# takah29/3d-reconstruction-from-multi-view-exp

Hardware: AMD Instinct MI355X
Metric: BA iterations/sec + residual-Jacobian GObs/s, 1M pts x 100 cams fp64 (higher is better)
Workload: dtype f64

## Files before the change

### 3d-reconstruction-from-multi-view-exp_amd/csrc/mvba.hip

```cpp
#include <dlfcn.h>
#include <hip/hip_runtime.h>
#include <rccl/rccl.h>

#include <algorithm>
#include <atomic>
#include <chrono>
#include <cmath>
#include <cstdlib>
#include <cstring>
#include <thread>
#include <type_traits>
#include <utility>
#include <vector>

#include "mvba_common.h"

namespace mvba {
thread_local std::string g_err;
}
using namespace mvba;

namespace {
struct Rccl {
  void *lib = nullptr;
  int version = 0;
  std::string origin;
  ncclResult_t (*GetVersion)(int *) = nullptr;
  ncclResult_t (*GetUniqueId)(ncclUniqueId *) = nullptr;
  ncclResult_t (*CommInitRank)(ncclComm_t *, int, ncclUniqueId, int) = nullptr;
  ncclResult_t (*CommDestroy)(ncclComm_t) = nullptr;
  ncclResult_t (*AllReduce)(const void *, void *, size_t, ncclDataType_t, ncclRedOp_t, ncclComm_t, hipStream_t) = nullptr;
  ncclResult_t (*AllGather)(const void *, void *, size_t, ncclDataType_t, ncclComm_t, hipStream_t) = nullptr;
  const char *(*GetErrorString)(ncclResult_t) = nullptr;
};
Rccl g_rccl;

int rccl_load() {
  if (g_rccl.lib) return MVBA_OK;
  const char *names[] = {"librccl.so.1", "librccl.so"};
  void *lib = nullptr;
  std::string origin;
  for (const char *n : names)
    if (!lib && (lib = dlopen(n, RTLD_NOW | RTLD_NOLOAD))) origin = std::string(n) + " (already mapped by the process)";
  if (const char *ev = getenv("MVBA_RCCL_LIBRARY"))
    if (!lib && (lib = dlopen(ev, RTLD_NOW | RTLD_GLOBAL))) origin = ev;
  for (const char *n : {"/opt/rocm/lib/librccl.so.1", "librccl.so.1"})
    if (!lib && (lib = dlopen(n, RTLD_NOW | RTLD_GLOBAL))) origin = n;
  if (!lib) return fail(MVBA_ERR_RCCL, std::string("librccl not found: ") + dlerror());
  Rccl r;
  r.lib = lib;
  r.origin = origin;
#define BIND(field, sym)                                                                       \
  if (!(r.field = reinterpret_cast<decltype(r.field)>(dlsym(lib, sym))))                       \
    return fail(MVBA_ERR_RCCL, std::string("librccl (") + origin + ") lacks " + sym)
  BIND(GetVersion, "ncclGetVersion");
  BIND(GetUniqueId, "ncclGetUniqueId");
  BIND(CommInitRank, "ncclCommInitRank");
  BIND(CommDestroy, "ncclCommDestroy");
  BIND(AllReduce, "ncclAllReduce");
  BIND(AllGather, "ncclAllGather");
  BIND(GetErrorString, "ncclGetErrorString");
#undef BIND
  if (r.GetVersion(&r.version) != ncclSuccess) return fail(MVBA_ERR_RCCL, "ncclGetVersion failed");
  const int major = r.version >= 10000 ? r.version / 10000 : r.version / 1000;
  if (major != NCCL_MAJOR)
    return fail(MVBA_ERR_RCCL, "librccl (" + origin + ") is NCCL " + std::to_string(r.version) + ", this library was built against " +
                                   std::to_string(NCCL_VERSION_CODE));
  g_rccl = r;
  return MVBA_OK;
}
}

namespace {

__device__ __forceinline__ double wave_sum(double v) {
#pragma unroll
  for (int off = 32; off > 0; off >>= 1) v += __shfl_down(v, off, 64);
  return v;
}

__device__ __forceinline__ double block_sum(double v, double *s_red ) {
  v = wave_sum(v);
  const int lane = threadIdx.x & 63, w = threadIdx.x >> 6;
  if (lane == 0) s_red[w] = v;
  __syncthreads();
  double t = 0.0;
  if (threadIdx.x == 0) {
    const int nw = (blockDim.x + 63) >> 6;
    for (int i = 0; i < nw; ++i) t += s_red[i];
  }
  return t;
}

__device__ __forceinline__ void load_cams_to_lds(const double *__restrict__ cam15, int m, double f0,
                                                 double *s_cam) {
  for (int k = threadIdx.x; k < m; k += blockDim.x) expand_cam(cam15 + (size_t)k * CAM_IN, f0, s_cam + k * CAM_LDS);
}

__host__ __device__ __forceinline__ size_t strip_offset(int k, int m) {
  return 81 * ((size_t)k * m - (size_t)k * (k - 1) / 2);
}

__device__ __forceinline__ int keep_index(int i, int gauge_axis) {
  if (i < 3) return i;
  return (i + 6 < 12 + gauge_axis) ? i + 6 : i + 7;
}

#define MVBA_CONST_AS __attribute__((address_space(4)))
template <typename T>
__device__ __forceinline__ const T MVBA_CONST_AS *as_const(const T *p) {
#pragma clang diagnostic push
#pragma clang diagnostic ignored "-Wold-style-cast"
  return (const T MVBA_CONST_AS *)p;
#pragma clang diagnostic pop
}

constexpr int REC = 8;
constexpr int LDS_CAMERAS = 646;

#define MVBA_RESID_JAC_ARGS                                                                                                 \
  long long nobs, int m, const double *__restrict__ cam15, const double *__restrict__ X, const int *__restrict__ obs_pt,   \
      const int *__restrict__ cam_idx, const double2 *__restrict__ xy, double f0, const int *__restrict__ tile_start,     \
      int n_tiles, double2 *__restrict__ rec, double *__restrict__ PL, const int *__restrict__ tile_slot,                 \
      double *__restrict__ PLsplit, const double *__restrict__ gcam
struct LossArgs {
  double b;
  double *sqw;
};
template <bool GCAM, int LOSS = LOSS_SQUARED, typename... Robust>
__global__ __launch_bounds__(1024, 4) void k_resid_jac(MVBA_RESID_JAC_ARGS, Robust... robust) {
  extern __shared__ __attribute__((aligned(16))) double smem[];
  double *s_cam = smem;
  const int lane = threadIdx.x & 63, wave = threadIdx.x >> 6, nwave = blockDim.x >> 6;
  double2 *stage = reinterpret_cast<double2 *>(smem + (GCAM ? 0 : ((m * CAM_LDS + 1) & ~1))) + wave * (64 * REC);
  constexpr int CS = 65;
  double *contrib = reinterpret_cast<double *>(stage);
  int *seg_start = reinterpret_cast<int *>(contrib + 9 * CS), *seg_pt = seg_start + 66;
  if (!GCAM) {
    load_cams_to_lds(cam15, m, f0, s_cam);
    __syncthreads();
  }
  for (int tile = blockIdx.x * nwave + wave; tile < n_tiles; tile += gridDim.x * nwave) {
    const int ts0 = tile_start[tile], ts1 = tile_start[tile + 1];
    const bool split = ts0 < 0;
    const int slot = split ? as_const(tile_slot)[tile] : 0;
    const long long wbase = split ? ~ts0 : ts0;
    const int n = (int)((ts1 < 0 ? ~ts1 : ts1) - wbase);
    const long long o = wbase + lane;
    const bool live = lane < n;
    int a = -1;
    double c9[9] = {0, 0, 0, 0, 0, 0, 0, 0, 0};
    if (live) {
      a = obs_pt[o];
      const int k = cam_idx[o];
      const double2 z = xy[o];
      const double *Xa = X + 3 * (size_t)a;
      ObsJ J;
      obs_math(Xa[0], Xa[1], Xa[2], GCAM ? gcam + (size_t)k * CAM_LDS : s_cam + k * CAM_LDS, z.x, z.y, f0, J);
      if constexpr (LOSS != LOSS_SQUARED) {
        const LossArgs la = (robust, ...);
        const double sw = loss_sqrt_w<LOSS>(J.e0 * J.e0 + J.e1 * J.e1, la.b);
        J.e0 *= sw;
        J.e1 *= sw;
#pragma unroll
        for (int rr = 0; rr < 2; ++rr) {
#pragma unroll
          for (int i = 0; i < 3; ++i) J.jx[rr][i] *= sw;
          J.jc[rr][0] *= sw;
#pragma unroll
          for (int i = 6; i < 9; ++i) J.jc[rr][i] *= sw;
        }
        la.sqw[o] = sw;
      }
      double2 *row = stage + lane * REC;
      const int sw = lane & 7;
      row[0 ^ sw] = make_double2(J.jx[0][0], J.jx[1][0]);
      row[1 ^ sw] = make_double2(J.jx[0][1], J.jx[1][1]);
      row[2 ^ sw] = make_double2(J.jx[0][2], J.jx[1][2]);
      row[3 ^ sw] = make_double2(J.jc[0][0], J.jc[1][0]);
      row[4 ^ sw] = make_double2(J.jc[0][6], J.jc[1][6]);
      row[5 ^ sw] = make_double2(J.jc[0][7], J.jc[1][7]);
      row[6 ^ sw] = make_double2(J.jc[0][8], J.jc[1][8]);
      row[7 ^ sw] = make_double2(J.e0, J.e1);
      c9[0] = 2.0 * (J.jx[0][0] * J.jx[0][0] + J.jx[1][0] * J.jx[1][0]);
      c9[1] = 2.0 * (J.jx[0][0] * J.jx[0][1] + J.jx[1][0] * J.jx[1][1]);
      c9[2] = 2.0 * (J.jx[0][0] * J.jx[0][2] + J.jx[1][0] * J.jx[1][2]);
      c9[3] = 2.0 * (J.jx[0][1] * J.jx[0][1] + J.jx[1][1] * J.jx[1][1]);
      c9[4] = 2.0 * (J.jx[0][1] * J.jx[0][2] + J.jx[1][1] * J.jx[1][2]);
      c9[5] = 2.0 * (J.jx[0][2] * J.jx[0][2] + J.jx[1][2] * J.jx[1][2]);
      c9[6] = 2.0 * (J.jx[0][0] * J.e0 + J.jx[1][0] * J.e1);
      c9[7] = 2.0 * (J.jx[0][1] * J.e0 + J.jx[1][1] * J.e1);
      c9[8] = 2.0 * (J.jx[0][2] * J.e0 + J.jx[1][2] * J.e1);
    }
    wave_sync();
#pragma unroll
    for (int q = 0; q < REC; ++q) {
      const int ol = q * 8 + (lane >> 3), pos = lane & 7;
      const double2 v = stage[ol * REC + pos];
      if (ol < n) rec[(wbase + ol) * REC + (pos ^ (ol & 7))] = v;
    }
    wave_sync();
    const int a_prev = __shfl_up(a, 1, 64);
    const bool head = live && (lane == 0 || a != a_prev);
    const unsigned long long heads = __ballot(head);
    const int nseg = __popcll(heads);
#pragma unroll
    for (int q = 0; q < 9; ++q) contrib[q * CS + lane] = c9[q];
    if (head) {
      const int rank = __popcll(heads & ((1ull << lane) - 1ull));
      seg_start[rank] = lane;
      seg_pt[rank] = a;
    }
    if (lane == 0) seg_start[nseg] = n;
    wave_sync();
    const int sl = lane / 9, comp = lane - 9 * sl;
    for (int s0 = 0; s0 < nseg; s0 += 7) {
      const int sg = s0 + sl;
      if (sl < 7 && sg < nseg) {
        const int i0 = seg_start[sg], i1 = seg_start[sg + 1];
        double acc = 0.0;
        for (int i = i0; i < i1; ++i) acc += contrib[comp * CS + i];
        if (split) PLsplit[9 * (size_t)slot + comp] = acc;
        else PL[9 * (size_t)seg_pt[sg] + comp] = acc;
      }
    }
    wave_sync();
  }
}

__global__ void k_sum_split(int n_split, const int4 *__restrict__ splits ,
                            const double *__restrict__ PLsplit, double *__restrict__ PL) {
  const int t = blockIdx.x * blockDim.x + threadIdx.x, sp = t / 9, comp = t - 9 * sp;
  if (sp >= n_split) return;
  const int4 d = splits[sp];
  double v = 0.0;
  for (int q = 0; q < d.z; ++q) v += PLsplit[9 * (size_t)(d.y + q) + comp];
  PL[9 * (size_t)d.x + comp] = v;
}

constexpr int PBS = 16;
constexpr int PACE_STRIDE = 32;
__global__ __launch_bounds__(256) void k_point_inv(long long npts, double c, const double *__restrict__ PL,
                                                   double *__restrict__ PB, int *__restrict__ flag,
                                                   double *__restrict__ Ab, long long nAb, int *__restrict__ prog, long long nprog, int want_r) {
  __shared__ double2 s_out[256 * 8];
  double *s_in = reinterpret_cast<double *>(s_out);
  const long long a0 = (long long)blockIdx.x * 256, a = a0 + threadIdx.x;
  for (long long i = a; i < nAb; i += (long long)gridDim.x * blockDim.x) Ab[i] = 0.0;
  for (long long i = a; i < nprog; i += (long long)gridDim.x * blockDim.x) prog[i] = 0;
  if (a0 >= npts) return;
  const int np = (int)min<long long>(256, npts - a0);
  {
    double t[9];
#pragma unroll
    for (int i = 0; i < 9; ++i) t[i] = PL[9 * a0 + min((int)threadIdx.x + 256 * i, 9 * np - 1)];
#pragma unroll
    for (int i = 0; i < 9; ++i)
      if ((int)threadIdx.x + 256 * i < 9 * np) s_in[threadIdx.x + 256 * i] = t[i];
  }
  __syncthreads();
  double in[9];
#pragma unroll
  for (int i = 0; i < 9; ++i) in[i] = s_in[9 * min((int)threadIdx.x, np - 1) + i];
  __syncthreads();
  if (threadIdx.x < np) {
    const double s = 1.0 + c;
    const double xx = in[0] * s, xy = in[1], xz = in[2], yy = in[3] * s, yz = in[4], zz = in[5] * s;
    const double c00 = yy * zz - yz * yz, c01 = xz * yz - xy * zz, c02 = xy * yz - xz * yy;
    const double det = xx * c00 + xy * c01 + xz * c02;
    if (!(det != 0.0) || !isfinite(det)) atomicOr(flag, 1);
    const double id = 1.0 / det;
    const double i00 = c00 * id, i01 = c01 * id, i02 = c02 * id;
    const double i11 = (xx * zz - xz * xz) * id, i12 = (xy * xz - xx * yz) * id, i22 = (xx * yy - xy * xy) * id;
    const double g0 = in[6], g1 = in[7], g2 = in[8];
    double2 *out = s_out + 8 * threadIdx.x;
    const int sw = threadIdx.x & 7;
    out[0 ^ sw] = make_double2(i00, i01);
    out[1 ^ sw] = make_double2(i02, i11);
    out[2 ^ sw] = make_double2(i12, i22);
    out[3 ^ sw] = make_double2(i00 * g0 + i01 * g1 + i02 * g2, i01 * g0 + i11 * g1 + i12 * g2);
    out[4 ^ sw] = make_double2(i02 * g0 + i12 * g1 + i22 * g2, 1.0);
    if (want_r) {
      const double d0 = i00, q0 = d0 != 0.0 ? 1.0 / d0 : 0.0, l10 = i01 * q0, l20 = i02 * q0;
      const double d1 = i11 - l10 * i01, q1 = d1 != 0.0 ? 1.0 / d1 : 0.0, l21 = (i12 - l20 * i01) * q1;
      const double d2 = i22 - l20 * i02 - l21 * l21 * d1;
      const double a0 = sqrt(fabs(d0)), a1 = sqrt(fabs(d1)), a2 = sqrt(fabs(d2));
      out[4 ^ sw].y = 1.0 + (d0 < 0.0 ? 1.0 : 0.0) + (d1 < 0.0 ? 2.0 : 0.0) + (d2 < 0.0 ? 4.0 : 0.0);
      out[5 ^ sw] = make_double2(a0, l10 * a0);
      out[6 ^ sw] = make_double2(l20 * a0, a1);
      out[7 ^ sw] = make_double2(l21 * a1, a2);
    } else {
      out[5 ^ sw] = out[6 ^ sw] = out[7 ^ sw] = make_double2(0.0, 0.0);
    }
  }
  __syncthreads();
  double2 *dst = reinterpret_cast<double2 *>(PB + PBS * a0);
  for (int e = threadIdx.x; e < 8 * np; e += 256) {
    const int p = e >> 3, sl = e & 7;
    dst[e] = s_out[8 * p + (sl ^ (p & 7))];
  }
}


constexpr int PSTEP = 21;
constexpr int PROW = 7 * 16;
constexpr int PWAVE_LDS = PSTEP * (2 * PROW + 5 * 16);
constexpr int UNIT_STRIDE = 104;
constexpr int SLOT_BUF = PSTEP * (2 * PROW + 3 * 16);
constexpr int SLOT_IDX = 64;
constexpr int SLOT_IDX_RING = 3;
constexpr int PAIRS_LDS = 2 * PWAVE_LDS;
constexpr int SLOT_LDS = 3 * SLOT_BUF + SLOT_IDX_RING * SLOT_IDX * 4;
static_assert(9 * ((SLOT_LDS + 511) / 512 * 512) <= 160 * 1024, "nine waves per CU");

__device__ __forceinline__ void lds_dma16(const void *gsrc, void *lds_wave_uniform) {
  __builtin_amdgcn_global_load_lds(gsrc, (__attribute__((address_space(3))) void *)lds_wave_uniform, 16, 0, 0);
}

struct SlotPace {
  const int *seg_end;
  int *prog;
  int need, nseg, lag;
};
template <bool DIAG, bool BIG, bool SLOTS = false, bool ROBUST = false>
__device__ __forceinline__ void schur_pairs_unit(char *wbuf, const int lane, const long long beg, const int n,
                                                 const int *__restrict__ it_k, const int *__restrict__ it_l,
                                                 const int *__restrict__ it_a, const double2 *__restrict__ rec,
                                                 const double *__restrict__ PB, const double c, const double cu,
                                                 double *__restrict__ out, const int *__restrict__ slot_unit = nullptr,
                                                 const SlotPace pace = SlotPace{nullptr, nullptr, 0, 0, 2},
                                                 const double *__restrict__ sqw = nullptr) {
  static_assert(!(SLOTS && ROBUST), "the slot form has no robust build");
  constexpr int NPS = DIAG ? 5 : 3;
  const int it = lane / 3, cg = lane - 3 * it;
  const int drow = lane / 7, dslot = lane - 7 * drow;
  const int prow = lane / NPS, pslot = lane - NPS * prow;
  const int prow2 = (64 + lane) / 5, pslot2 = (64 + lane) - 5 * prow2;
  const int sel0 = cg == 0 ? 3 : (cg == 1 ? 0 : 4);
  const int sel1 = cg == 0 ? 0 : sel0 + 1, sel2 = cg == 0 ? 0 : sel0 + 2;
  const double al12 = cg == 0 ? 0.0 : 1.0, bx1 = cg == 0 ? 1.0 : 0.0;
  double acc[9][3];
#pragma unroll
  for (int i = 0; i < 9; ++i)
#pragma unroll
    for (int q = 0; q < 3; ++q) acc[i][q] = 0.0;
  double dg[3] = {0.0, 0.0, 0.0}, rb[3] = {0.0, 0.0, 0.0};

  constexpr int LB_OFF = PSTEP * PROW;
  constexpr int PB_OFF = LB_OFF + ((SLOTS && DIAG) ? PSTEP * 16 : PSTEP * PROW);
  constexpr int BUFSZ = SLOTS ? PB_OFF + PSTEP * 16 * NPS : PWAVE_LDS;
  static_assert(!SLOTS || BUFSZ <= SLOT_BUF, "slot form: staging buffer larger than the launch provides");
  constexpr int W_OFF = DIAG ? LB_OFF + PSTEP * 16 : PB_OFF + PSTEP * 16 * NPS;
  static_assert(!ROBUST || (DIAG ? W_OFF + PSTEP * 8 <= PB_OFF : W_OFF + 2 * PSTEP * 8 <= BUFSZ), "robust weights fit the staging buffer");
  int ixk[1][3], ixl[1][3], ixa[1][2];
  int ixw[2] = {0, 0};
  auto load_idx = [&](int s0, int (&xk)[3], int (&xl)[3], int (&xa)[2]) {
    const unsigned last = (unsigned)(min(PSTEP, n - s0) - 1);
    typedef const int __attribute__((address_space(1))) *gint_p;
    auto uni = [](const int *p) {
      const unsigned long long v = (unsigned long long)p;
      const unsigned lo = __builtin_amdgcn_readfirstlane((unsigned)v), hi = __builtin_amdgcn_readfirstlane((unsigned)(v >> 32));
      return (gint_p)(((unsigned long long)hi << 32) | lo);
    };
    typedef const char __attribute__((address_space(1))) *gchar_p;
    auto row_of = [&](int r) {
      unsigned off = min((unsigned)r, last) << 2;
      asm("" : "+v"(off));
      return off;
    };
    auto at = [](gint_p base, unsigned off) { return *(gint_p)((gchar_p)base + off); };
    const gint_p pk = uni(it_k + (beg + s0)), pl = DIAG ? pk : uni(it_l + (beg + s0)), pa = uni(it_a + (beg + s0));
#pragma unroll
    for (int q = 0; q < 3; ++q) {
      const unsigned row = row_of(9 * q + drow);
      xk[q] = at(pk, row);
      if (!DIAG) xl[q] = at(pl, row);
    }
    if (DIAG) xl[0] = at(pk, row_of(lane));
    xa[0] = at(pa, row_of(prow));
    if (DIAG) xa[1] = at(pa, row_of(prow2));
    if (ROBUST) {
      ixw[0] = at(pk, row_of(lane >> 1));
      if (!DIAG) ixw[1] = at(pl, row_of(lane >> 1));
    }
  };
  auto rec_at = [&](int obs, int slot) -> const void * {
    if (BIG) return rec + (size_t)obs * REC + slot;
    return reinterpret_cast<const char *>(rec) + (((unsigned)obs << 7) + ((unsigned)slot << 4));
  };
  auto pb_at = [&](int a, int slot) -> const void * {
    if (BIG) return PB + (size_t)a * PBS + 2 * slot;
    return reinterpret_cast<const char *>(PB) + (((unsigned)a << 7) + ((unsigned)slot << 4));
  };
  auto issue = [&](char *buf, const int (&xk_)[3], const int (&xl_)[3], const int (&xa_)[2]) {
    char *kb = buf, *lb = buf + LB_OFF, *pb_ = buf + PB_OFF;
    const int (&xk)[3] = xk_, (&xl)[3] = xl_, (&xa)[2] = xa_;
    if (lane < 63) {
#pragma unroll
      for (int q = 0; q < 2; ++q) {
        lds_dma16(rec_at(xk[q], dslot), kb + q * (9 * PROW));
        if (!DIAG) lds_dma16(rec_at(xl[q], dslot), lb + q * (9 * PROW));
      }
      if (!DIAG) lds_dma16(pb_at(xa[0], pslot), pb_);
    }
    if (lane < 7 * (PSTEP - 18)) {
      lds_dma16(rec_at(xk[2], dslot), kb + 2 * (9 * PROW));
      if (!DIAG) lds_dma16(rec_at(xl[2], dslot), lb + 2 * (9 * PROW));
    }
    if (DIAG) {
      if (lane < PSTEP) lds_dma16(rec_at(xl[0], 7), lb);
      lds_dma16(pb_at(xa[0], pslot), pb_);
      if (lane < 5 * PSTEP - 64) lds_dma16(pb_at(xa[1], pslot2), pb_ + 1024);
    }
    if (ROBUST && lane < 2 * PSTEP) {
      const char *wsrc = reinterpret_cast<const char *>(sqw) + (lane & 1) * 4;
      __builtin_amdgcn_global_load_lds(wsrc + (size_t)ixw[0] * 8, (__attribute__((address_space(3))) void *)(buf + W_OFF), 4, 0, 0);
      if (!DIAG)
        __builtin_amdgcn_global_load_lds(wsrc + (size_t)ixw[1] * 8, (__attribute__((address_space(3))) void *)(buf + W_OFF + PSTEP * 8), 4, 0, 0);
    }
  };
  auto compute = [&](const char *buf, const int ns) {
    const char *kbuf = buf, *lbuf = buf + LB_OFF, *pbuf = buf + PB_OFF;
    if (it < ns) {
      double swk = 1.0, swl = 1.0;
      if (ROBUST) {
        const double *wl = reinterpret_cast<const double *>(buf + W_OFF);
        swk = wl[it];
        swl = DIAG ? swk : wl[PSTEP + it];
      }
      const double2 *kr = reinterpret_cast<const double2 *>(kbuf + it * PROW);
      const double2 *lr = DIAG ? kr : reinterpret_cast<const double2 *>(lbuf + it * PROW);
      const double *pb = reinterpret_cast<const double *>(pbuf + it * (16 * NPS));
      const double2 kx0 = kr[0], kx1 = kr[1], kx2 = kr[2], kf = kr[3], kw0 = kr[4], kw1 = kr[5], kw2 = kr[6];
      const double2 lx0 = lr[0], lx1 = lr[1], lx2 = lr[2];
      const double i00 = pb[0], i01 = pb[1], i02 = pb[2], i11 = pb[3], i12 = pb[4], i22 = pb[5];
      const double h0x = i00 * lx0.x + i01 * lx1.x + i02 * lx2.x, h0y = i00 * lx0.y + i01 * lx1.y + i02 * lx2.y;
      const double h1x = i01 * lx0.x + i11 * lx1.x + i12 * lx2.x, h1y = i01 * lx0.y + i11 * lx1.y + i12 * lx2.y;
      const double h2x = i02 * lx0.x + i12 * lx1.x + i22 * lx2.x, h2y = i02 * lx0.y + i12 * lx1.y + i22 * lx2.y;
      double t00 = kx0.x * h0x + kx1.x * h1x + kx2.x * h2x, t01 = kx0.x * h0y + kx1.x * h1y + kx2.x * h2y;
      double t10 = kx0.y * h0x + kx1.y * h1x + kx2.y * h2x, t11 = kx0.y * h0y + kx1.y * h1y + kx2.y * h2y;
      double w0 = 0.0, w1 = 0.0;
      const double wgt = (DIAG && SLOTS) ? pb[9] : 1.0;
      if (DIAG) {
        t00 -= SLOTS ? 0.5 * wgt : 0.5;
        t11 -= SLOTS ? 0.5 * wgt : 0.5;
        const double2 e = reinterpret_cast<const double2 *>(lbuf)[it];
        w0 = kx0.x * pb[6] + kx1.x * pb[7] + kx2.x * pb[8] - e.x;
        w1 = kx0.y * pb[6] + kx1.y * pb[7] + kx2.y * pb[8] - e.y;
        if (SLOTS) {
          w0 *= wgt;
          w1 *= wgt;
        }
      }
      const double2 s0v = lr[sel0], s1v = lr[sel1], s2v = lr[sel2];
      const double bxw = ROBUST ? bx1 * swl : bx1;
      const double sx[3] = {s0v.x, al12 * s1v.x + bxw, al12 * s2v.x};
      const double sy[3] = {s0v.y, al12 * s1v.y, al12 * s2v.y + bxw};
#pragma unroll
      for (int q = 0; q < 3; ++q) {
        const double v0 = t00 * sx[q] + t01 * sy[q], v1 = t10 * sx[q] + t11 * sy[q];
        acc[0][q] = fma(kf.y, v1, fma(kf.x, v0, acc[0][q]));
        if (ROBUST) {
          acc[1][q] = fma(swk, v0, acc[1][q]);
          acc[2][q] = fma(swk, v1, acc[2][q]);
        } else {
          acc[1][q] += v0;
          acc[2][q] += v1;
        }
        acc[3][q] = fma(kx0.y, v1, fma(kx0.x, v0, acc[3][q]));
        acc[4][q] = fma(kx1.y, v1, fma(kx1.x, v0, acc[4][q]));
        acc[5][q] = fma(kx2.y, v1, fma(kx2.x, v0, acc[5][q]));
        acc[6][q] = fma(kw0.y, v1, fma(kw0.x, v0, acc[6][q]));
        acc[7][q] = fma(kw1.y, v1, fma(kw1.x, v0, acc[7][q]));
        acc[8][q] = fma(kw2.y, v1, fma(kw2.x, v0, acc[8][q]));
        if (DIAG) {
          if (SLOTS) dg[q] = fma(wgt, sx[q] * sx[q] + sy[q] * sy[q], dg[q]);
          else dg[q] += sx[q] * sx[q] + sy[q] * sy[q];
          rb[q] += sx[q] * w0 + sy[q] * w1;
        }
      }
    }
    asm volatile("s_waitcnt lgkmcnt(0)" ::: "memory");
  };
  bool pacing = SLOTS;
  int seg = 0, seg_stop = pacing ? as_const(pace.seg_end)[0] * PSTEP : 0x7fffffff;
  auto pace_at = [&](const int s0) {
    while (s0 == seg_stop) {
      if (lane == 0) __hip_atomic_fetch_add(pace.prog + PACE_STRIDE * seg, 1, __ATOMIC_RELAXED, __HIP_MEMORY_SCOPE_AGENT);
      ++seg;
      seg_stop = seg < pace.nseg ? as_const(pace.seg_end)[seg] * PSTEP : 0x7fffffff;
      if (seg >= pace.lag && pacing) {
        int tries = 0;
        while (__hip_atomic_fetch_add(pace.prog + PACE_STRIDE * (seg - pace.lag), 0, __ATOMIC_RELAXED, __HIP_MEMORY_SCOPE_AGENT) < pace.need) {
          if (++tries > 1024) { pacing = false; break; }
          __builtin_amdgcn_s_sleep(127);
        }
        if (tries > 0) __builtin_amdgcn_s_setprio(0);
        else __builtin_amdgcn_s_setprio(2);
      }
    }
  };
  if (!SLOTS) {
    load_idx(0, ixk[0], ixl[0], ixa[0]);
    issue(wbuf, ixk[0], ixl[0], ixa[0]);
    if (PSTEP < n) load_idx(PSTEP, ixk[0], ixl[0], ixa[0]);
    for (int s0 = 0, par = 0; s0 < n; s0 += PSTEP, par ^= 1) {
      const int ns = min(PSTEP, n - s0);
      asm volatile("s_waitcnt vmcnt(0)" ::: "memory");
      if (s0 + PSTEP < n) {
        issue(wbuf + (par ^ 1) * BUFSZ, ixk[0], ixl[0], ixa[0]);
        if (s0 + 2 * PSTEP < n) load_idx(s0 + 2 * PSTEP, ixk[0], ixl[0], ixa[0]);
      }
      compute(wbuf + par * BUFSZ, ns);
    }
  } else {
    constexpr int SLOT_OPS = DIAG ? 7 : 8;
    const int nst = n / PSTEP, last_st = nst - 1;
    const unsigned lds0 = (unsigned)(unsigned long long)(__attribute__((address_space(3))) char *)wbuf;
    const unsigned ldsx0 = lds0 + 3 * SLOT_BUF;
    const int *xring = reinterpret_cast<const int *>(wbuf + 3 * SLOT_BUF);
    const int *xbase = it_k + beg * SLOT_IDX;
    static_assert(!SLOTS || !BIG, "the slot form has no 64-bit-offset build");
    auto dma = [&](int row, unsigned slot16, const void *base, unsigned lds) {
      unsigned o;
      asm volatile("s_mov_b32 m0, %4\n\tv_lshl_add_u32 %0, %1, 7, %2\n\tglobal_load_lds_dwordx4 %0, %3" : "=&v"(o) : "v"(row), "v"(slot16), "s"(base), "s"(lds) : "memory");
    };
    const unsigned lane16 = (unsigned)min(lane, 15) << 4;
    auto dma_idx = [&](int st, unsigned ring_off) {
      const int *src = xbase + (size_t)min(st, last_st) * SLOT_IDX;
// ... 1621 lines not shown
  for (int k = threadIdx.x; k < m; k += blockDim.x) {
    const double *Kk = K + 9 * (size_t)k, *Rk = R + 9 * (size_t)k, *tk = t + 3 * (size_t)k;
    double Rt[3][4];
    for (int i = 0; i < 3; ++i) {
      for (int j = 0; j < 3; ++j) Rt[i][j] = Rk[3 * j + i];
      Rt[i][3] = -(Rt[i][0] * tk[0] + Rt[i][1] * tk[1] + Rt[i][2] * tk[2]);
    }
    for (int i = 0; i < 3; ++i)
      for (int j = 0; j < 4; ++j) sP[12 * k + 4 * i + j] = Kk[3 * i] * Rt[0][j] + Kk[3 * i + 1] * Rt[1][j] + Kk[3 * i + 2] * Rt[2][j];
  }
  __syncthreads();
  const long long stride = (long long)gridDim.x * blockDim.x;
  for (long long o = (long long)blockIdx.x * blockDim.x + threadIdx.x; o < nobs; o += stride) {
    const long long a = obs_pt ? obs_pt[o] : o / m;
    const int k = cam_idx ? cam_idx[o] : (int)(o - a * m);
    const double *Xa = X + 3 * a, *P = sP + 12 * k;
    const double p0 = Xa[0] * P[0] + Xa[1] * P[1] + Xa[2] * P[2] + P[3];
    const double p1 = Xa[0] * P[4] + Xa[1] * P[5] + Xa[2] * P[6] + P[7];
    const double p2 = Xa[0] * P[8] + Xa[1] * P[9] + Xa[2] * P[10] + P[11];
    xy[o] = make_double2(p0 / p2, p1 / p2);
  }
}

__global__ __launch_bounds__(256) void k_similarity(long long npts, int m, double *__restrict__ X, double *__restrict__ cam15,
                                                    const double *__restrict__ T13) {
  const double *R0 = T13, *t0 = T13 + 9;
  const double s = T13[12];
  const long long a = (long long)blockIdx.x * blockDim.x + threadIdx.x;
  if (a < npts) {
    double *x = X + 3 * a;
    const double x0 = s * x[0], x1 = s * x[1], x2 = s * x[2];
#pragma unroll
    for (int i = 0; i < 3; ++i) x[i] = x0 * R0[3 * i] + x1 * R0[3 * i + 1] + x2 * R0[3 * i + 2] + t0[i];
  }
  if (a < m) {
    double *c = cam15 + (size_t)a * CAM_IN;
    const double p0 = s * c[3], p1 = s * c[4], p2 = s * c[5];
    double Rn[9];
#pragma unroll
    for (int i = 0; i < 3; ++i) {
#pragma unroll
      for (int j = 0; j < 3; ++j) Rn[3 * i + j] = R0[3 * i] * c[6 + j] + R0[3 * i + 1] * c[9 + j] + R0[3 * i + 2] * c[12 + j];
    }
#pragma unroll
    for (int i = 0; i < 3; ++i) c[3 + i] = p0 * R0[3 * i] + p1 * R0[3 * i + 1] + p2 * R0[3 * i + 2] + t0[i];
#pragma unroll
    for (int i = 0; i < 9; ++i) c[6 + i] = Rn[i];
  }
}

constexpr int IDX_WAVES = 4;

__device__ __forceinline__ int idx_pair_id(int k, int l, int m) { return k * m - k * (k - 1) / 2 + (l - k); }

template <bool GLOBAL>
__global__ __launch_bounds__(64 * IDX_WAVES) void k_idx_count(long long N, int m, int P, const long long *__restrict__ pt_ptr,
                                                              const int *__restrict__ cam_idx, int chunk,
                                                              int *__restrict__ hist, const int *__restrict__ order) {
  extern __shared__ int s_hist_all[];
  const int lane = threadIdx.x & 63, wv = threadIdx.x >> 6;
  const long long w = (long long)blockIdx.x * IDX_WAVES + wv;
  int *s_hist = GLOBAL ? hist + (size_t)w * P : s_hist_all + (size_t)wv * P;
  if (!GLOBAL) {
    for (int q = lane; q < P; q += 64) s_hist[q] = 0;
    wave_sync();
  }
  const long long a0 = w * chunk, a1 = min(N, a0 + chunk);
  for (long long ai = a0; ai < a1; ++ai) {
    const long long a = order ? order[ai] : ai;
    const long long o0 = pt_ptr[a];
    const int d = (int)(pt_ptr[a + 1] - o0);
    for (int i = 0; i < d; ++i) {
      const int k = cam_idx[o0 + i];
      for (int j = i + lane; j < d; j += 64) {
        int *c = s_hist + idx_pair_id(k, cam_idx[o0 + j], m);
        if (GLOBAL) __hip_atomic_store(c, __hip_atomic_load(c, __ATOMIC_RELAXED, __HIP_MEMORY_SCOPE_AGENT) + 1, __ATOMIC_RELAXED, __HIP_MEMORY_SCOPE_AGENT);
        else *c += 1;
      }
      wave_sync();
    }
  }
  if (!GLOBAL)
    for (int q = lane; q < P; q += 64) hist[(size_t)w * P + q] = s_hist[q];
}

__global__ void k_idx_scan(int P, int n_waves, int *__restrict__ hist, long long *__restrict__ cnt) {
  const int q = blockIdx.x * blockDim.x + threadIdx.x;
  if (q >= P) return;
  long long run = 0;
  for (int w = 0; w < n_waves; ++w) {
    const int v = hist[(size_t)w * P + q];
    hist[(size_t)w * P + q] = (int)run;
    run += v;
  }
  cnt[q] = run;
}

template <bool GLOBAL>
__global__ __launch_bounds__(64 * IDX_WAVES) void k_idx_fill(long long N, int m, int P, const long long *__restrict__ pt_ptr,
                                                             const int *__restrict__ cam_idx, int chunk,
                                                             int *__restrict__ hist, const int *__restrict__ S,
                                                             const int *__restrict__ vp_ptr, const long long *__restrict__ vp_off,
                                                             int *__restrict__ it_k, int *__restrict__ it_l, int *__restrict__ it_a,
                                                             const int *__restrict__ order) {
  extern __shared__ int s_hist_all[];
  const int lane = threadIdx.x & 63, wv = threadIdx.x >> 6;
  const long long w = (long long)blockIdx.x * IDX_WAVES + wv;
  int *s_rank = GLOBAL ? hist + (size_t)w * P : s_hist_all + (size_t)wv * P;
  if (!GLOBAL) {
    for (int q = lane; q < P; q += 64) s_rank[q] = hist[(size_t)w * P + q];
    wave_sync();
  }
  const long long a0 = w * chunk, a1 = min(N, a0 + chunk);
  for (long long ai = a0; ai < a1; ++ai) {
    const long long a = order ? order[ai] : ai;
    const long long o0 = pt_ptr[a];
    const int d = (int)(pt_ptr[a + 1] - o0);
    for (int i = 0; i < d; ++i) {
      const int k = cam_idx[o0 + i];
      for (int j = i + lane; j < d; j += 64) {
        const int q = idx_pair_id(k, cam_idx[o0 + j], m);
        int r;
        if (GLOBAL) {
          r = __hip_atomic_load(s_rank + q, __ATOMIC_RELAXED, __HIP_MEMORY_SCOPE_AGENT);
          __hip_atomic_store(s_rank + q, r + 1, __ATOMIC_RELAXED, __HIP_MEMORY_SCOPE_AGENT);
        } else {
          r = s_rank[q];
          s_rank[q] = r + 1;
        }
        const int sq = S[q];
        const long long pos = vp_off[vp_ptr[q] + (r % sq)] + r / sq;
        it_k[pos] = (int)(o0 + i);
        it_l[pos] = (int)(o0 + j);
        it_a[pos] = (int)a;
      }
      wave_sync();
    }
  }
}

__global__ void k_idx_bounds(int VP, int nR, const long long *__restrict__ vp_off, const long long *__restrict__ range_lo,
                             const int *__restrict__ it_a, long long *__restrict__ lo, const int *__restrict__ rank) {
  const long long t = (long long)blockIdx.x * blockDim.x + threadIdx.x;
  if (t >= (long long)VP * (nR + 1)) return;
  const int v = (int)(t / (nR + 1)), r = (int)(t - (long long)v * (nR + 1));
  long long b = vp_off[v], e = vp_off[v + 1];
  const long long key = range_lo[r];
  while (b < e) {
    const long long mid = (b + e) >> 1;
    if ((rank ? rank[it_a[mid]] : it_a[mid]) < key) b = mid + 1;
    else e = mid;
  }
  lo[t] = b;
}

template <bool FILL>
__global__ __launch_bounds__(64) void k_idx_merge(long long n_waves, int nR, int nSeg, long long skew, long long segG,
                                                  const long long *__restrict__ sl_beg, const int *__restrict__ sl_len,
                                                  const long long *__restrict__ range_o0, const int *__restrict__ it_k,
                                                  const int *__restrict__ it_l, const int *__restrict__ it_a,
                                                  const long long *__restrict__ w_beg, int pad_obs, int pad_pt,
                                                  int *__restrict__ w_steps, int *__restrict__ st_k, int *__restrict__ st_l,
                                                  int *__restrict__ st_a, int *__restrict__ seg_end, const long long *__restrict__ pkey) {
  const long long b = blockIdx.x;
  const int lane = threadIdx.x;
  const bool slot = lane < PSTEP;
  long long cur = slot ? sl_beg[b * PSTEP + lane] : 0;
  const long long end = slot ? cur + sl_len[b * PSTEP + lane] : 0;
  const long long o_lo = range_o0[b % nR];
  const long long base = FILL ? w_beg[b] : 0;
  constexpr long long NONE = 1LL << 40;
  int steps = 0, sg = 0;
  auto key_at = [&](long long c) -> long long { return pkey[it_a[c]]; };
  long long k0 = cur < end ? key_at(cur) : NONE, k1 = cur + 1 < end ? key_at(cur + 1) : NONE;
  while (true) {
    long long lo = k0;
#pragma unroll
    for (int off = 32; off > 0; off >>= 1) lo = min(lo, __shfl_xor(lo, off, 64));
    if (FILL && lo < NONE && lane == 0)
      while (sg < nSeg && lo >= o_lo + (sg + 1) * segG) seg_end[b * nSeg + sg++] = steps;
    if (lo >= NONE) break;
    const bool take = k0 < NONE && k0 <= lo + skew;
    if (FILL && slot) {
      const long long o = (base + steps) * PSTEP + lane;
      st_k[o] = take ? (int)(it_k[cur] - o_lo) : pad_obs;
      st_l[o] = take ? (int)(it_l[cur] - o_lo) : pad_obs;
      st_a[o] = take ? it_a[cur] : pad_pt;
    }
    if (take) {
      ++cur;
      k0 = k1;
      k1 = cur + 1 < end ? key_at(cur + 1) : NONE;
    }
    ++steps;
  }
  if (FILL) {
    if (lane == 0)
      while (sg < nSeg) seg_end[b * nSeg + sg++] = steps;
  } else if (lane == 0) {
    w_steps[b] = steps;
  }
}

__global__ void k_idx_interleave(long long n_steps, const int *__restrict__ st_k, const int *__restrict__ st_l, const int *__restrict__ st_a,
                                 int *__restrict__ out) {
  const long long t = (long long)blockIdx.x * blockDim.x + threadIdx.x;
  if (t >= n_steps * SLOT_IDX) return;
  const long long st = t / SLOT_IDX;
  const int e = (int)(t - st * SLOT_IDX), which = e / PSTEP, sl = e - which * PSTEP;
  const int *src = which == 0 ? st_k : (which == 1 ? st_l : st_a);
  out[t] = which < 3 ? src[st * PSTEP + sl] : 0;
}

#include "mvba_cov.h"
#include "mvba_map.h"

}

struct DevBufs {
  std::vector<void *> bufs;
  DevBufs() = default;
  DevBufs(const DevBufs &) = delete;
  DevBufs &operator=(const DevBufs &) = delete;
  ~DevBufs() { release_all(); }
  template <typename T>
  int alloc(T **p, size_t n) {
    const size_t bytes = std::max<size_t>(n, 1) * sizeof(T);
    const hipError_t e = hipMalloc((void **)p, bytes);
    if (e != hipSuccess) {
      size_t fr = 0, tot = 0;
      hipMemGetInfo(&fr, &tot);
      *p = nullptr;
      return fail(MVBA_ERR_HIP, std::string("hipMalloc of ") + std::to_string(bytes) + " bytes: " + hipGetErrorString(e) + " (" + std::to_string(fr >> 20) +
                                    " MiB free of " + std::to_string(tot >> 20) + ")");
    }
    bufs.push_back(*p);
    return MVBA_OK;
  }
  void own(void *q) { bufs.push_back(q); }
  bool forget(void *q) {
    auto it = std::find(bufs.begin(), bufs.end(), q);
    if (it == bufs.end()) return false;
    bufs.erase(it);
    return true;
  }
  template <typename T>
  void release(T *&p) {
    if (p && forget(p)) hipFree(p);
    p = nullptr;
  }
  template <typename T>
  void adopt(DevBufs &from, T *p) {
    if (p && from.forget(p)) bufs.push_back(p);
  }
  void release_all() {
    for (void *q : bufs) hipFree(q);
    bufs.clear();
  }
};

enum { SCHUR_PAIRS = 1, SCHUR_SLOTS = 2, SCHUR_DENSE = 3 };
struct mvba_handle {
  int device = 0;
  hipStream_t stream = nullptr;
  DevBufs mem;
  long long N = 0, nobs = 0;
  int m = 0, gauge_axis = 0, D = 0, ld = 0;
  double f0 = 1.0;
  long long *d_pt_ptr = nullptr;
  int *d_cam = nullptr, *d_obs_pt = nullptr;
  double2 *d_xy = nullptr;
  int *d_tiles = nullptr;
  int *d_tile_slot = nullptr;
  int4 *d_splits = nullptr;
  double *d_PLsplit = nullptr;
  int n_splits = 0;
  int n_tiles = 0;
  bool any_split = false;
  int k1_threads = 512;
  bool use_pairs = true;
  int schur_mode = 2;
  long long n_items = 0, n_items_offdiag = 0, n_slot_items = 0;
  int n_units = 0, rccl_version = 0, q_max = 0, n_waves = 0, slot_nR = 8, slot_nseg = 0;
  long long *d_range_o0 = nullptr;
  int *d_seg_end = nullptr, *d_prog = nullptr;
  bool check_solve = false;
  double check_solve_tol = 1e-8;
  bool gcam = false;
  double *d_cam18 = nullptr, *d_dxi10 = nullptr;
  bool index_on_device = false;
  int4 *d_wdesc = nullptr;
  int *d_it_x = nullptr;
  int *d_wunits = nullptr;
  bool force_big = false;
  int *d_it_k = nullptr, *d_it_l = nullptr, *d_it_a = nullptr, *d_unit_ptr = nullptr, *d_q_ptr = nullptr, *d_q_units = nullptr;
  int4 *d_units = nullptr;
  double *d_partial = nullptr;
  double *d_dense_part = nullptr;
  int *d_dense_obs = nullptr;
  int dense_blocks = 0, dense_tiles = 0;
  double *d_X[2] = {nullptr, nullptr}, *d_cam15[2] = {nullptr, nullptr};
  int cur = 0;
  bool have_params = false, linearized = false, have_trial = false;
  double2 *d_rec = nullptr;
  double *d_PL = nullptr, *d_PB = nullptr;
  double *d_Ab = nullptr, *d_Ared = nullptr, *d_Ztiles = nullptr, *d_Lblk = nullptr, *d_dxi = nullptr, *d_dX = nullptr, *d_lu = nullptr;
  int *d_ipiv = nullptr;
  double *d_partials = nullptr, *d_cost = nullptr, *h_cost = nullptr;
  double *d_mail = nullptr;
  unsigned long long cost_seq = 0;
  bool mail_pending = false;
  int n_partials = 0, cost_grid = 0;
  int *d_flag = nullptr, *h_flag = nullptr;
  unsigned *d_bar = nullptr;
  int n_cu = 1;
  bool chol_onepass = true;
  int trail64_min = 200;
  unsigned barrier_polls = 1u << 22;
  ncclComm_t comm = nullptr;
  mvba_host_allreduce_fn host_ar = nullptr;
  void *host_ar_user = nullptr;
  std::vector<double> host_buf;
  int rank = 0, nranks = 1;
  double *d_allcost = nullptr, *h_allcost = nullptr, *d_sim = nullptr;
  std::vector<double *> snap_slabs;
  long long n_snap = 0;
  int profiling = 0;
  mvba_stats stats{};
  struct Ev { int kid; hipEvent_t a, b; };
  std::vector<Ev> pending;
  std::vector<hipEvent_t> pool;
  double *d_cov_sig = nullptr, *d_cov_panel = nullptr, *d_cov_pts = nullptr, *d_cov_cam = nullptr;
  int loss = LOSS_SQUARED;
  double loss_b = 0.0;
  double *d_sqw = nullptr;
  double2 *d_resid = nullptr;
  double *d_init_cams = nullptr;
  bool mapped = false;
  int n_free = 0, map_ld = 0, map_U = 0;
  std::vector<int> map_col, map_ptr, map_mem;
  int *d_map_col = nullptr, *d_map_ptr = nullptr, *d_map_mem = nullptr;
  double *d_map_x = nullptr, *d_cov_sigv = nullptr;
  int2 *d_map_pairs = nullptr;
  double *d_map_part = nullptr;
  int n_map_pairs = 0, map_nblk = 1;
  int solve_D() const { return mapped ? n_free : D; }
  int solve_ld() const { return mapped ? map_ld : ld; }
};

namespace {

const char *kKernelNames[MVBA_K_COUNT] = {"resid_jac", "point_blocks", "point_inv", "schur",
                                          "allreduce", "solve",        "backsub_cost", "cost"};

struct Timed {
  mvba_handle *h;
  int kid;
  hipEvent_t a = nullptr, b = nullptr;
  bool on = false;
  Timed(mvba_handle *h_, int kid_) : h(h_), kid(kid_) {
    on = kid >= 0 && (h->profiling == 1 || (h->profiling == 2 && (kid == MVBA_K_SCHUR || kid == MVBA_K_RESID_JAC)));
    if (!on) return;
    auto get = [&]() {
      hipEvent_t e;
      if (!h->pool.empty()) { e = h->pool.back(); h->pool.pop_back(); }
      else hipEventCreate(&e);
      return e;
    };
    a = get(); b = get();
    hipEventRecord(a, h->stream);
  }
  ~Timed() {
    if (!on) return;
    hipEventRecord(b, h->stream);
    h->pending.push_back({kid, a, b});
  }
};

void drain_events(mvba_handle *h) {
  for (auto &p : h->pending) {
    float ms = 0.f;
    if (hipEventElapsedTime(&ms, p.a, p.b) == hipSuccess) {
      h->stats.ms[p.kid] += ms;
      h->stats.launches[p.kid] += 1;
    }
    h->pool.push_back(p.a);
    h->pool.push_back(p.b);
  }
  h->pending.clear();
}

int sync_and_drain(mvba_handle *h) {
  MVBA_HIP(hipStreamSynchronize(h->stream));
  drain_events(h);
  return MVBA_OK;
}

inline void cpu_relax() {
#if defined(__x86_64__) && !defined(__HIP_DEVICE_COMPILE__)
  __builtin_ia32_pause();
#endif
}

double *cost_mail(mvba_handle *h) {
  if (h->comm || h->host_ar || h->profiling == 1 || !h->d_mail) return nullptr;
  ++h->cost_seq;
  h->mail_pending = true;
  return h->d_mail;
}

int global_cost(mvba_handle *h, double *E) {
  if (h->mail_pending) {
    h->mail_pending = false;
    volatile unsigned long long *seq = reinterpret_cast<volatile unsigned long long *>(h->h_cost + 2);
    const auto t0 = std::chrono::steady_clock::now();
    bool seen = false;
    for (unsigned spins = 0;; ++spins) {
      if (*seq == h->cost_seq) { seen = true; break; }
      if ((spins & 1023) == 1023 && std::chrono::steady_clock::now() - t0 > std::chrono::seconds(2)) break;
      cpu_relax();
    }
    if (seen) {
      std::atomic_thread_fence(std::memory_order_acquire);
      drain_events(h);
      *E = h->h_cost[0];
      return MVBA_OK;
    }
    int rc = sync_and_drain(h);
    if (rc) return rc;
    *E = h->h_cost[0];
    return MVBA_OK;
  }
  if (h->comm) {
    Timed t(h, MVBA_K_ALLREDUCE);
    ncclResult_t r = g_rccl.AllGather(h->d_cost, h->d_allcost, 2, ncclDouble, h->comm, h->stream);
    if (r != ncclSuccess) return fail(MVBA_ERR_RCCL, std::string("ncclAllGather: ") + g_rccl.GetErrorString(r));
    MVBA_HIP(hipMemcpyAsync(h->h_allcost, h->d_allcost, 2 * sizeof(double) * h->nranks, hipMemcpyDeviceToHost, h->stream));
  } else {
    MVBA_HIP(hipMemcpyAsync(h->h_cost, h->d_cost, 2 * sizeof(double), hipMemcpyDeviceToHost, h->stream));
  }
  int rc = sync_and_drain(h);
  if (rc) return rc;
  if (h->host_ar) {
    std::vector<double> v(2 * (size_t)h->nranks, 0.0);
    v[2 * h->rank] = h->h_cost[0];
    v[2 * h->rank + 1] = (double)*h->h_flag;
    if (h->host_ar(h->host_ar_user, v.data(), (int64_t)v.size())) return fail(MVBA_ERR_RCCL, "host all-reduce callback failed");
    double s = 0.0;
    int fl = 0;
    for (int i = 0; i < h->nranks; ++i) { s += v[2 * i]; fl |= (int)v[2 * i + 1]; }
    *E = s;
    *h->h_flag = fl;
  } else if (h->comm) {
    double s = 0.0;
    int fl = 0;
    for (int i = 0; i < h->nranks; ++i) {
      s += h->h_allcost[2 * i];
      int f;
      memcpy(&f, &h->h_allcost[2 * i + 1], sizeof(int));
      fl |= f;
    }
    *E = s;
    *h->h_flag = fl;
  } else {
    *E = *h->h_cost;
  }
  return MVBA_OK;
}

template <typename... A>
struct LossKernel {
  void (*squared)(A...);
  void (*robust)(A..., LossArgs);
  const void *fn(bool rb) const { return rb ? (const void *)robust : (const void *)squared; }
};
template <typename... A>
LossKernel<A...> loss_kernel(void (*squared)(A...), void (*robust)(A..., LossArgs)) { return {squared, robust}; }

template <typename... A, typename... Args>
void launch_loss(mvba_handle *h, LossKernel<A...> k, dim3 grid, dim3 block, size_t lds, Args... args) {
  if (h->loss != LOSS_SQUARED) hipLaunchKernelGGL(k.robust, grid, block, lds, h->stream, args..., LossArgs{h->loss_b, h->d_sqw});
  else hipLaunchKernelGGL(k.squared, grid, block, lds, h->stream, args...);
}

auto resid_jac_kernel(bool gcam, int loss) {
  if (loss == LOSS_CAUCHY)
    return gcam ? loss_kernel(k_resid_jac<true>, k_resid_jac<true, LOSS_CAUCHY, LossArgs>) : loss_kernel(k_resid_jac<false>, k_resid_jac<false, LOSS_CAUCHY, LossArgs>);
  return gcam ? loss_kernel(k_resid_jac<true>, k_resid_jac<true, LOSS_HUBER, LossArgs>) : loss_kernel(k_resid_jac<false>, k_resid_jac<false, LOSS_HUBER, LossArgs>);
}
auto cost_kernel(bool gcam, int loss) {
  if (loss == LOSS_CAUCHY)
    return gcam ? loss_kernel(k_cost<true>, k_cost<true, LOSS_CAUCHY, LossArgs>) : loss_kernel(k_cost<false>, k_cost<false, LOSS_CAUCHY, LossArgs>);
  return gcam ? loss_kernel(k_cost<true>, k_cost<true, LOSS_HUBER, LossArgs>) : loss_kernel(k_cost<false>, k_cost<false, LOSS_HUBER, LossArgs>);
}
template <int G>
auto backsub_kernel_g(int bt, bool gcam) {
  if (gcam) return loss_kernel(k_backsub<G, 256, true>, k_backsub<G, 256, true, true, LossArgs>);
  if (bt == 1024) return loss_kernel(k_backsub<G, 1024>, k_backsub<G, 1024, false, true, LossArgs>);
  if (bt == 512) return loss_kernel(k_backsub<G, 512>, k_backsub<G, 512, false, true, LossArgs>);
  return loss_kernel(k_backsub<G>, k_backsub<G, 256, false, true, LossArgs>);
}
auto backsub_kernel(int G, int bt, bool gcam) {
  return G == 2 ? backsub_kernel_g<2>(bt, gcam) : (G == 4 ? backsub_kernel_g<4>(bt, gcam) : backsub_kernel_g<8>(bt, gcam));
}
template <int T>
auto dense_kernel_t(bool table) {
  return table ? loss_kernel(k_schur_dense<T, true>, k_schur_dense<T, true, true, LossArgs>)
               : loss_kernel(k_schur_dense<T, false>, k_schur_dense<T, false, true, LossArgs>);
}
auto dense_kernel(int T, bool table) {
  switch (T) {
    case 1: return dense_kernel_t<1>(table);
    case 2: return dense_kernel_t<2>(table);
    case 3: return dense_kernel_t<3>(table);
    case 4: return dense_kernel_t<4>(table);
    case 5: return dense_kernel_t<5>(table);
    case 6: return dense_kernel_t<6>(table);
    case 7: return dense_kernel_t<7>(table);
    case 8: return dense_kernel_t<8>(table);
    case 9: return dense_kernel_t<9>(table);
    case 10: return dense_kernel_t<10>(table);
    case 11: return dense_kernel_t<11>(table);
    default: return dense_kernel_t<12>(table);
  }
}
size_t dense_lds_bytes(int T, int mm) {
  const int CH = dense_ch(T);
  return sizeof(double) * ((size_t)2 * 3 * CH * 16 * T + (size_t)2 * CH * mm * 32) + sizeof(double2) * CH * ((size_t)mm * REC + 8) +
         sizeof(double) * (CH * (size_t)mm + 2 * 3 * CH);
}

size_t k1_lds_bytes(int m, bool gcam, int threads) {
  return (size_t)((gcam ? 0 : ((m * CAM_LDS + 1) & ~1)) + (threads / 64) * 64 * 2 * REC) * sizeof(double);
}
size_t cam_lds_bytes(int m, bool gcam, bool with_dxi) { return gcam ? 0 : (size_t)m * (CAM_LDS + (with_dxi ? DXI_LDS : 0)) * sizeof(double); }

void cam_tables(mvba_handle *h, const double *cam15, const double *dxi) {
  if (h->gcam) hipLaunchKernelGGL(k_cam_tables, dim3((h->m + 255) / 256), dim3(256), 0, h->stream, h->m, cam15, dxi, h->f0, h->d_cam18, h->d_dxi10);
}
int launch_cost(mvba_handle *h, const double *cam15, const double *X) {
  const size_t lds = cam_lds_bytes(h->m, h->gcam, false);
  cam_tables(h, cam15, nullptr);
  launch_loss(h, cost_kernel(h->gcam, h->loss), dim3(h->cost_grid), dim3(lds > 40 * 1024 ? 512 : 256), lds, h->nobs, h->m, cam15, X,
              h->d_obs_pt, h->d_cam, h->d_xy, h->f0, h->d_partials, h->d_cam18);
  double *mail = cost_mail(h);
  const unsigned long long seq = h->cost_seq;
  hipLaunchKernelGGL(k_sum_partials, dim3(1), dim3(1024), 0, h->stream, h->d_partials, h->cost_grid, h->d_cost, h->d_flag, mail, seq);
  MVBA_HIP(hipGetLastError());
  return MVBA_OK;
}

struct CreateKnobs {
  bool schur_set = false;
  bool schur_slots = false, schur_pairs = false, schur_dense = false;
  bool index_host = false, index_global = false;
  bool force_big = false;
  bool chol_launches = false;
  int trail64_min = 200;
  unsigned barrier_polls = 1u << 22;
  bool check_solve = false;
  double check_solve_tol = 1e-8;
  bool timing = false;
};

CreateKnobs read_create_knobs() {
  CreateKnobs k;
  auto is = [](const char *ev, const char *v) { return ev && !strcmp(ev, v); };
  const char *schur = getenv("MVBA_SCHUR");
  k.schur_set = schur != nullptr;
  k.schur_slots = is(schur, "slots");
  k.schur_pairs = is(schur, "pairs");
  k.schur_dense = is(schur, "dense");
  const char *index = getenv("MVBA_INDEX");
  k.index_host = is(index, "host");
  k.index_global = is(index, "global");
  k.force_big = getenv("MVBA_FORCE_BIG") != nullptr;
  k.chol_launches = is(getenv("MVBA_CHOL"), "launches");
  if (const char *ev = getenv("MVBA_TRAIL64_MIN")) k.trail64_min = std::max(0, atoi(ev));
  if (const char *ev = getenv("MVBA_CHOL_BARRIER_POLLS")) k.barrier_polls = (unsigned)std::max(0LL, atoll(ev));
  if (const char *ev = getenv("MVBA_CHECK_SOLVE")) {
    const double v = atof(ev);
    k.check_solve = v != 0.0;
    if (v > 0.0 && v < 1.0) k.check_solve_tol = v;
  }
  k.timing = getenv("MVBA_CREATE_TIMING") != nullptr;
  return k;
}

#include "mvba_create.h"

}

extern "C" {

const char *mvba_version(void) { return "mvba 0.2 (gfx950)"; }
const char *mvba_last_error(void) { return g_err.c_str(); }
const char *mvba_kernel_name(int32_t k) { return (k >= 0 && k < MVBA_K_COUNT) ? kKernelNames[k] : ""; }

int mvba_device_count(int32_t *count) {
  int n = 0;
  hipError_t e = hipGetDeviceCount(&n);
  if (e != hipSuccess) {
    *count = 0;
    return fail(MVBA_ERR_HIP, std::string("hipGetDeviceCount: ") + hipGetErrorString(e));
  }
  *count = n;
  return MVBA_OK;
}

int mvba_create(const mvba_problem *p, mvba_handle **out) { return create_engine(p, LOSS_SQUARED, 0.0, out); }

int mvba_create_robust(const mvba_problem *p, int32_t loss, double scale, mvba_handle **out) {
  if (!p || !out) return fail(MVBA_ERR_BADARG, "null argument");
  if (loss == LOSS_SQUARED) return create_engine(p, LOSS_SQUARED, 0.0, out);
  if (loss != LOSS_HUBER && loss != LOSS_CAUCHY)
    return fail(MVBA_ERR_BADARG, "loss = " + std::to_string(loss) + " is not a loss (0 squared, 1 Huber, 2 Cauchy)");
  if (!(scale > 0.0) || !std::isfinite(scale))
    return fail(MVBA_ERR_BADARG, "loss scale = " + std::to_string(scale) + " must be finite and > 0 for a robust loss");
  if (!(p->f0 > 0.0) || !std::isfinite(p->f0)) return fail(MVBA_ERR_BADARG, "a robust loss needs f0 > 0");
  const double r = scale / p->f0;
  return create_engine(p, loss, r * r, out);
}

void mvba_destroy(mvba_handle *h) {
  if (!h) return;
  hipSetDevice(h->device);
  if (h->stream) hipStreamSynchronize(h->stream);
  if (h->comm) g_rccl.CommDestroy(h->comm);
  h->mem.release_all();
  if (h->h_cost) hipHostFree(h->h_cost);
  if (h->h_allcost) hipHostFree(h->h_allcost);
  for (auto &p : h->pending) { hipEventDestroy(p.a); hipEventDestroy(p.b); }
  for (auto e : h->pool) hipEventDestroy(e);
  if (h->stream) hipStreamDestroy(h->stream);
  delete h;
}

int mvba_set_params(mvba_handle *h, const double *X, const double *f, const double *u, const double *t, const double *R) {
  if (!h || !X || !f || !u || !t || !R) return fail(MVBA_ERR_BADARG, "null argument");
  MVBA_HIP(hipSetDevice(h->device));
  std::vector<double> cam((size_t)h->m * CAM_IN);
  for (int k = 0; k < h->m; ++k) {
    double *c = cam.data() + (size_t)k * CAM_IN;
    c[0] = f[k]; c[1] = u[2 * k]; c[2] = u[2 * k + 1];
    for (int i = 0; i < 3; ++i) c[3 + i] = t[3 * k + i];
    for (int i = 0; i < 9; ++i) c[6 + i] = R[9 * k + i];
  }
  MVBA_HIP(hipMemcpyAsync(h->d_X[h->cur], X, sizeof(double) * 3 * h->N, hipMemcpyHostToDevice, h->stream));
  MVBA_HIP(hipMemcpyAsync(h->d_cam15[h->cur], cam.data(), sizeof(double) * cam.size(), hipMemcpyHostToDevice, h->stream));
  MVBA_HIP(hipStreamSynchronize(h->stream));
  h->have_params = true; h->linearized = false; h->have_trial = false;
  return MVBA_OK;
}

int mvba_get_params(mvba_handle *h, double *X, double *f, double *u, double *t, double *R) {
  if (!h || !X || !f || !u || !t || !R) return fail(MVBA_ERR_BADARG, "null argument");
  if (!h->have_params) return fail(MVBA_ERR_STATE, "no parameters set");
  MVBA_HIP(hipSetDevice(h->device));
  std::vector<double> cam((size_t)h->m * CAM_IN);
  MVBA_HIP(hipMemcpyAsync(X, h->d_X[h->cur], sizeof(double) * 3 * h->N, hipMemcpyDeviceToHost, h->stream));
  MVBA_HIP(hipMemcpyAsync(cam.data(), h->d_cam15[h->cur], sizeof(double) * cam.size(), hipMemcpyDeviceToHost, h->stream));
  MVBA_HIP(hipStreamSynchronize(h->stream));
  for (int k = 0; k < h->m; ++k) {
    const double *c = cam.data() + (size_t)k * CAM_IN;
    f[k] = c[0]; u[2 * k] = c[1]; u[2 * k + 1] = c[2];
    for (int i = 0; i < 3; ++i) t[3 * k + i] = c[3 + i];
    for (int i = 0; i < 9; ++i) R[9 * k + i] = c[6 + i];
  }
  return MVBA_OK;
}

int mvba_apply_similarity(mvba_handle *h, const double *R0, const double *t0, double scale) {
  if (!h || !R0 || !t0) return fail(MVBA_ERR_BADARG, "null argument");
  if (!h->have_params) return fail(MVBA_ERR_STATE, "no parameters set");
  MVBA_HIP(hipSetDevice(h->device));
  double T[13];
  memcpy(T, R0, 9 * sizeof(double));
  memcpy(T + 9, t0, 3 * sizeof(double));
  T[12] = scale;
  if (!h->d_sim) {
    int rc = h->mem.alloc(&h->d_sim, 13);
    if (rc) return rc;
  }
  MVBA_HIP(hipMemcpyAsync(h->d_sim, T, sizeof(T), hipMemcpyHostToDevice, h->stream));
  const long long n = std::max<long long>(h->N, h->m);
  hipLaunchKernelGGL(k_similarity, dim3((unsigned)((n + 255) / 256)), dim3(256), 0, h->stream, h->N, h->m, h->d_X[h->cur],
                     h->d_cam15[h->cur], h->d_sim);
  MVBA_HIP(hipGetLastError());
  MVBA_HIP(hipStreamSynchronize(h->stream));
  h->linearized = false; h->have_trial = false;
  return MVBA_OK;
}

int mvba_cost(mvba_handle *h, double *E) {
  if (!h || !E) return fail(MVBA_ERR_BADARG, "null argument");
  if (!h->have_params) return fail(MVBA_ERR_STATE, "no parameters set");
  MVBA_HIP(hipSetDevice(h->device));
  {
    Timed t(h, MVBA_K_COST);
    int rc = launch_cost(h, h->d_cam15[h->cur], h->d_X[h->cur]);
    if (rc) return rc;
  }
  return global_cost(h, E);
}

namespace {
void launch_resid_jac(mvba_handle *h) {
  const int kt = h->k1_threads;
  cam_tables(h, h->d_cam15[h->cur], nullptr);
  const int wpb = kt / 64;
  const int grid = std::max(1, std::min(2048 * 256 / kt, (h->n_tiles + wpb - 1) / wpb));
  launch_loss(h, resid_jac_kernel(h->gcam, h->loss), dim3(grid), dim3(kt), k1_lds_bytes(h->m, h->gcam, kt), h->nobs, h->m, h->d_cam15[h->cur],
              h->d_X[h->cur], h->d_obs_pt, h->d_cam, h->d_xy, h->f0, h->d_tiles, h->n_tiles, h->d_rec, h->d_PL,
              h->d_tile_slot, h->d_PLsplit, h->d_cam18);
  if (h->n_splits)
    hipLaunchKernelGGL(k_sum_split, dim3((9 * h->n_splits + 255) / 256), dim3(256), 0, h->stream, h->n_splits, h->d_splits,
                       h->d_PLsplit, h->d_PL);
}

void launch_point_inv(mvba_handle *h, double c) {
  const int m = h->m;
  const size_t n9 = 9 * (size_t)m, nA = strip_offset(m, m);
  const long long nAb = (long long)(nA + n9);
  const unsigned grid = (unsigned)std::max<long long>((h->N + 255) / 256, std::min<long long>((nAb + 1023) / 1024, 4096));
  hipLaunchKernelGGL(k_point_inv, dim3(std::max(grid, 1u)), dim3(256), 0, h->stream, h->N, c, h->d_PL, h->d_PB, h->d_flag,
                     h->d_Ab, nAb, h->d_prog, (long long)h->slot_nR * h->slot_nseg * PACE_STRIDE,
                     h->schur_mode == SCHUR_DENSE ? 1 : 0);
}

void launch_schur(mvba_handle *h, double c) {
  const int m = h->m;
  const size_t nA = strip_offset(m, m);
  double *d_A = h->d_Ab, *d_b = h->d_Ab + nA;
  if (h->use_pairs) {
    const bool big = (std::max<long long>(h->nobs, h->N) + 1) * 128LL >= (1LL << 32) || h->force_big;
    if (h->schur_mode == SCHUR_SLOTS) {
      if (h->n_waves)
        hipLaunchKernelGGL(k_schur_slots, dim3(h->n_waves), dim3(64), SLOT_LDS, h->stream, h->d_wdesc,
                           h->d_wunits, h->d_it_x, (const int *)nullptr, (const int *)nullptr, h->d_rec, h->d_PB, c, h->f0, h->d_partial,
                           h->slot_nR, h->d_seg_end, h->d_prog, h->slot_nseg, SLOT_LAG, h->d_range_o0);
    } else if (h->n_units) {
      auto launch = [&](auto kern, auto... robust) {
        hipLaunchKernelGGL(kern, dim3(8 * h->q_max), dim3(64), PAIRS_LDS, h->stream, h->d_units, h->d_q_ptr, h->d_q_units, h->d_it_k, h->d_it_l,
                           h->d_it_a, h->d_rec, h->d_PB, c, h->f0, h->d_partial, robust...);
      };
      if (h->loss != LOSS_SQUARED) launch(big ? k_schur_pairs_big_robust : k_schur_pairs_robust, (const double *)h->d_sqw);
      else launch(big ? k_schur_pairs_big : k_schur_pairs);
    }
    hipLaunchKernelGGL(k_schur_reduce, dim3((unsigned)((long long)m * (m + 1) / 2)), dim3(128), 0, h->stream, m, h->d_unit_ptr,
                       h->d_partial, d_A, d_b);
  } else if (h->schur_mode == SCHUR_DENSE) {
    const int T = (9 * m + 15) / 16;
    launch_loss(h, dense_kernel(T, h->d_dense_obs != nullptr), dim3(h->dense_blocks), dim3(64 * (dense_consumers(T) + dense_ch(T))), dense_lds_bytes(T, m),
                (const double2 *)h->d_rec, (const double *)h->d_PB, (const int *)h->d_dense_obs, (long long)h->N, m, 1.0 / h->f0, h->d_dense_part);
    const long long n_el = (long long)nA + 9 * m;
    hipLaunchKernelGGL(k_schur_dense_finish, dim3((unsigned)((n_el + 3) / 4)), dim3(256), 0, h->stream, m, T, h->dense_blocks,
                       (const double *)h->d_dense_part, c, d_A, d_b);
  }
}

int allreduce_Ab(mvba_handle *h, bool timed) {
  const int m = h->m;
  const size_t n9 = 9 * (size_t)m, nA = strip_offset(m, m);
  if (h->comm) {
    Timed t(h, timed ? MVBA_K_ALLREDUCE : -1);
    ncclResult_t r = g_rccl.AllReduce(h->d_Ab, h->d_Ab, nA + n9, ncclDouble, ncclSum, h->comm, h->stream);
    if (r != ncclSuccess) return fail(MVBA_ERR_RCCL, std::string("ncclAllReduce: ") + g_rccl.GetErrorString(r));
  } else if (h->host_ar) {
    h->host_buf.resize(nA + n9);
    MVBA_HIP(hipMemcpyAsync(h->host_buf.data(), h->d_Ab, sizeof(double) * (nA + n9), hipMemcpyDeviceToHost, h->stream));
    MVBA_HIP(hipStreamSynchronize(h->stream));
    const auto t0 = std::chrono::steady_clock::now();
    if (h->host_ar(h->host_ar_user, h->host_buf.data(), (int64_t)(nA + n9))) return fail(MVBA_ERR_RCCL, "host all-reduce callback failed");
    MVBA_HIP(hipMemcpyAsync(h->d_Ab, h->host_buf.data(), sizeof(double) * (nA + n9), hipMemcpyHostToDevice, h->stream));
    if (timed && h->profiling) {
      h->stats.ms[MVBA_K_ALLREDUCE] += std::chrono::duration<double, std::milli>(std::chrono::steady_clock::now() - t0).count();
      h->stats.launches[MVBA_K_ALLREDUCE] += 1;
    }
  }
  return MVBA_OK;
}

void launch_map_tied(mvba_handle *h, double *M, int ld, int mirror) {
  if (!h->n_map_pairs) return;
  hipLaunchKernelGGL(k_map_tied, dim3(h->n_map_pairs, h->map_nblk), dim3(256), 0, h->stream, h->m, (const double *)h->d_Ab,
                     (const int *)h->d_map_ptr, (const int *)h->d_map_mem, (const int2 *)h->d_map_pairs, h->d_map_part);
  hipLaunchKernelGGL(k_map_tied_finish, dim3((h->n_map_pairs + 255) / 256), dim3(256), 0, h->stream, h->n_map_pairs, h->map_nblk, ld,
                     mirror, (const int2 *)h->d_map_pairs, (const double *)h->d_map_part, M);
}

void launch_factor(mvba_handle *h) {
  const int m = h->m, D = h->solve_D();
  double *d_A = h->d_Ab, *d_b = h->d_Ab + strip_offset(m, m);
  const int ld = h->solve_ld();
  const int ntc = (D + NB - 1) / NB;
  if (h->mapped) {
    const int U = h->map_U, ntu = (U + NB - 1) / NB;
    hipLaunchKernelGGL(k_map_compact, dim3(ntu * (ntu + 1) / 2 + (D + 255) / 256), dim3(256), 0, h->stream, D, ld, m, U, ntu, d_A, d_b,
                       h->d_map_ptr, h->d_map_mem, h->d_Ared, h->d_bar, 1 + 4 * ((D + SBW - 1) / SBW));
    if (U < D)
      hipLaunchKernelGGL(k_map_rows, dim3((D + 63) / 64, D - U), dim3(256), 0, h->stream, D, ld, m, U, d_A, h->d_map_ptr, h->d_map_mem,
                         h->d_Ared);
    launch_map_tied(h, h->d_Ared, ld, 0);
  } else
  hipLaunchKernelGGL(k_compact, dim3(ntc * (ntc + 1) / 2 + (D + 255) / 256), dim3(256), 0, h->stream, D, ld, m, h->gauge_axis, ntc, d_A, d_b,
                     h->d_Ared, h->d_bar, 1 + 4 * ((D + SBW - 1) / SBW));
  for (int jS = 0; jS < D; jS += SBW) {
    const int jE = std::min(jS + SBW, D);
    hipLaunchKernelGGL(k_chol_super, dim3((D + 1 - jE + 63) / 64), dim3(SUPER_THREADS), SUPER_LDS, h->stream, h->d_Ared, ld, D, jS,
                       h->d_Ztiles + (size_t)(jS / NB) * NB * NB, h->d_Lblk + (size_t)(jS / SBW) * SBW * SBW, h->d_flag);
    if (jE < D) {
      const int nt32 = (D + 1 - jE + NB - 1) / NB, nt64 = (D + 1 - jE + TB - 1) / TB;
      if (jE - jS == SBW && nt64 * (nt64 + 1) / 2 >= h->trail64_min)
        hipLaunchKernelGGL(k_chol_trail64, dim3(nt64 * (nt64 + 1) / 2), dim3(256), TRAIL64_LDS, h->stream, h->d_Ared, ld, D, jS, jE);
      else
        hipLaunchKernelGGL(k_chol_trail32, dim3(nt32 * (nt32 + 1) / 2), dim3(256), 0, h->stream, h->d_Ared, ld, D, jS, jE);
    }
  }
}
}

int mvba_linearize(mvba_handle *h) {
  if (!h) return fail(MVBA_ERR_BADARG, "null handle");
  if (!h->have_params) return fail(MVBA_ERR_STATE, "no parameters set");
  MVBA_HIP(hipSetDevice(h->device));
  if (h->nobs) {
    Timed t(h, MVBA_K_RESID_JAC);
    launch_resid_jac(h);
  }
  MVBA_HIP(hipGetLastError());
  h->linearized = true; h->have_trial = false;
  h->stats.n_linearize++;
  return MVBA_OK;
}

namespace {
double *solve_x(mvba_handle *h) { return h->mapped ? h->d_map_x : h->d_dxi; }
void launch_expand(mvba_handle *h) {
  const size_t n9 = 9 * (size_t)h->m;
  if (h->mapped && h->solve_D() > 0)
    hipLaunchKernelGGL(k_map_expand, dim3((unsigned)((n9 + 255) / 256)), dim3(256), 0, h->stream, (int)n9, h->gauge_axis, h->d_map_col,
                       h->d_map_x, h->d_dxi);
}

void launch_solve(mvba_handle *h, bool onepass) {
  const int m = h->m, D = h->solve_D();
  double *d_x = solve_x(h);
  Timed t(h, MVBA_K_SOLVE);
  if (D == 0) {
    hipMemsetAsync(h->d_dxi, 0, sizeof(double) * 9 * (size_t)m, h->stream);
    return;
  }
  launch_factor(h);
  const int ld = h->solve_ld();
  const int S = (D + SBW - 1) / SBW;
  if (onepass && (S == 1 || S < h->n_cu)) {
    const int ngrp = ((S - 1) * SBW + 31) / 32, nbulk = S > 1 ? std::max(1, std::min(h->n_cu - S, ngrp)) : 0;
    hipLaunchKernelGGL(k_chol_backsolve_all<true>, dim3(S + nbulk), dim3(SUPER_THREADS),
                       BACKSOLVE_LDS, h->stream, h->d_Ared, ld, D, m, h->gauge_axis, h->d_Ztiles, h->d_Lblk, d_x, h->d_flag,
                       h->d_bar, h->barrier_polls);
  } else
  for (int jS = ((D - 1) / SBW) * SBW; jS >= 0; jS -= SBW) {
    const int jE = std::min(jS + SBW, D), jE2 = std::min(jE + SBW, D);
    const int nwg = (jE == D) ? 1 : 1 + (jS + 255) / 256;
    hipLaunchKernelGGL(k_chol_backsolve, dim3(nwg), dim3(256), 0, h->stream, h->d_Ared, ld, D, m, h->gauge_axis, h->d_Ztiles,
                       h->d_Lblk + (size_t)(jS / SBW) * SBW * SBW, d_x, jS, jE, jE2);
  }
  launch_expand(h);
}

int launch_lu_solve(mvba_handle *h) {
  const int m = h->m, D = h->solve_D();
  double *d_A = h->d_Ab, *d_b = h->d_Ab + strip_offset(m, m), *d_x = solve_x(h);
  if (!h->d_lu) {
    int rc_ = h->mem.alloc(&h->d_lu, (size_t)h->D * (h->D + 1));
    if (rc_) return rc_;
    rc_ = h->mem.alloc(&h->d_ipiv, (size_t)h->D);
    if (rc_) return rc_;
  }
  MVBA_HIP(hipMemsetAsync(h->d_flag, 0, sizeof(int), h->stream));
  Timed t(h, MVBA_K_SOLVE);
  if (h->mapped) {
    hipLaunchKernelGGL(k_map_full, dim3((D + 1 + 255) / 256, D), dim3(256), 0, h->stream, D, m, d_A, d_b, h->d_map_ptr, h->d_map_mem, h->d_lu);
    launch_map_tied(h, h->d_lu, D + 1, 1);
  } else
  hipLaunchKernelGGL(k_compact_full, dim3((D + 1 + 255) / 256, D), dim3(256), 0, h->stream, D, m, h->gauge_axis, d_A, d_b, h->d_lu);
  for (int j0 = 0; j0 < D; j0 += LU_NB) {
    const int nb = std::min(LU_NB, D - j0), right = D + 1 - (j0 + nb);
    hipLaunchKernelGGL(k_lu_panel, dim3(1), dim3(1024), 0, h->stream, h->d_lu, D, j0, nb, h->d_ipiv, h->d_flag);
    hipLaunchKernelGGL(k_lu_swap, dim3((D + 1 - nb + 255) / 256), dim3(256), 0, h->stream, h->d_lu, D, j0, nb, h->d_ipiv);
    if (right > 0) hipLaunchKernelGGL(k_lu_trsm, dim3((right + 255) / 256), dim3(256), 0, h->stream, h->d_lu, D, j0, nb);
    const int below = D - (j0 + nb);
    if (below > 0)
      hipLaunchKernelGGL(k_lu_gemm, dim3((right + 63) / 64, (below + 63) / 64), dim3(256), 0, h->stream, h->d_lu, D, j0, nb);
  }
  hipLaunchKernelGGL(k_lu_backsub, dim3(1), dim3(1024), 0, h->stream, h->d_lu, D, m, h->gauge_axis, d_x);
  launch_expand(h);
  return MVBA_OK;
}

int launch_tail_and_cost(mvba_handle *h, double *E_trial) {
  const int m = h->m, trial = 1 - h->cur;
  {
    Timed t(h, MVBA_K_BACKSUB_COST);
    hipLaunchKernelGGL(k_update_cams, dim3((m + 63) / 64), dim3(64), 0, h->stream, m, h->d_cam15[h->cur], h->d_dxi,
                       h->d_cam15[trial]);
    if (h->N) {
      const size_t lds = cam_lds_bytes(m, h->gcam, true);
      cam_tables(h, h->d_cam15[h->cur], h->d_dxi);
      const double deg = (double)h->nobs / (double)h->N;
      const int G = deg <= 40.0 ? 2 : (deg <= 100.0 ? 4 : 8);
      const int bt = lds > 80 * 1024 ? 1024 : (lds > 40 * 1024 ? 512 : 256);
      const int nblk = (int)std::min<long long>(4096 * 256 / bt, (h->N * G + bt - 1) / bt);
      launch_loss(h, backsub_kernel(G, bt, h->gcam), dim3(nblk), dim3(bt), lds, h->N, m, h->d_pt_ptr, h->d_cam, h->d_PB, h->d_dxi,
                  h->d_X[h->cur], h->d_cam15[h->cur], h->f0, h->d_X[trial], h->d_dX, h->d_cam18, h->d_dxi10);
    }
    int rc = launch_cost(h, h->d_cam15[trial], h->d_X[trial]);
    if (rc) return rc;
  }
  return global_cost(h, E_trial);
}

int check_solve_residual(mvba_handle *h) {
  const int m = h->m, D = h->solve_D();
  const size_t n9 = 9 * (size_t)m, nA = strip_offset(m, m);
  std::vector<double> Ab(nA + n9), x(n9);
  MVBA_HIP(hipMemcpyAsync(Ab.data(), h->d_Ab, sizeof(double) * (nA + n9), hipMemcpyDeviceToHost, h->stream));
  MVBA_HIP(hipMemcpyAsync(x.data(), h->d_dxi, sizeof(double) * n9, hipMemcpyDeviceToHost, h->stream));
  MVBA_HIP(hipStreamSynchronize(h->stream));
  auto kept = [&](size_t g) { return !((g >= 3 && g <= 8) || g == (size_t)(12 + h->gauge_axis)); };
  std::vector<double> r(n9, 0.0), an(n9, 0.0);
  for (int k = 0; k < m; ++k) {
    const double *Ak = Ab.data() + strip_offset(k, m);
    const int Wk = 9 * (m - k);
    for (int i = 0; i < 9; ++i)
      for (int c = 0; c < Wk; ++c) {
        const size_t gi = 9 * (size_t)k + i, gj = 9 * (size_t)k + c;
        const double a = Ak[(size_t)i * Wk + c];
        r[gi] += a * x[gj]; an[gi] += std::fabs(a * x[gj]);
        if (c >= 9) { r[gj] += a * x[gi]; an[gj] += std::fabs(a * x[gi]); }
      }
  }
  double worst = 0.0;
  if (h->mapped) {
    for (int j = 0; j < D; ++j) {
      double res = 0.0, scale = 0.0;
      for (int q = h->map_ptr[j]; q < h->map_ptr[j + 1]; ++q) {
        const size_t g = (size_t)h->map_mem[q];
        res += Ab[nA + g] - r[g];
        scale += an[g] + std::fabs(Ab[nA + g]);
      }
      worst = std::max(worst, scale > 0.0 ? std::fabs(res) / scale : 0.0);
    }
  } else
  for (size_t g = 0; g < n9; ++g)
    if (kept(g)) {
      const double bg = Ab[nA + g], scale = an[g] + std::fabs(bg);
      worst = std::max(worst, scale > 0.0 ? std::fabs(bg - r[g]) / scale : 0.0);
    }
  if (!(worst <= h->check_solve_tol))
    return fail(MVBA_ERR_STATE, "MVBA_CHECK_SOLVE: the dense solve left a relative residual of " + std::to_string(worst) +
                                    " on the reduced camera system (a stale hand-over in the back-substitution?)");
  return MVBA_OK;
}
}

int mvba_try_step(mvba_handle *h, double c, double *E_trial) {
  if (!h || !E_trial) return fail(MVBA_ERR_BADARG, "null argument");
  if (!h->linearized) return fail(MVBA_ERR_STATE, "try_step before linearize");
  MVBA_HIP(hipSetDevice(h->device));
  {
    Timed t(h, MVBA_K_POINT_INV);
    launch_point_inv(h, c);
  }
  if (h->use_pairs || h->schur_mode == SCHUR_DENSE) {
    Timed t(h, MVBA_K_SCHUR);
    launch_schur(h, c);
  }
  MVBA_HIP(hipGetLastError());
  int rc = allreduce_Ab(h, true);
  if (rc) return rc;
  launch_solve(h, h->chol_onepass);
  MVBA_HIP(hipGetLastError());
  h->stats.n_try_step++;
  rc = launch_tail_and_cost(h, E_trial);
  if (rc) return rc;
  if ((*h->h_flag & 8) && !(*h->h_flag & 1)) {
    MVBA_HIP(hipMemsetAsync(h->d_flag, 0, sizeof(int), h->stream));
    h->chol_onepass = false;
    h->stats.n_barrier_fallback++;
    launch_solve(h, false);
    rc = launch_tail_and_cost(h, E_trial);
    if (rc) return rc;
  }
  if ((*h->h_flag & 2) && !(*h->h_flag & (1 | 8))) {
    rc = launch_lu_solve(h);
    if (rc) return rc;
    h->stats.n_lu_fallback++;
    rc = launch_tail_and_cost(h, E_trial);
    if (rc) return rc;
  }
  if (*h->h_flag) {
    const int fl = *h->h_flag;
    hipMemsetAsync(h->d_flag, 0, sizeof(int), h->stream);
    if (fl & 8) return fail(MVBA_ERR_HIP, "k_chol_backsolve_all: a wait for a progress word timed out twice (is another process holding the CUs?)");
    return fail(MVBA_ERR_SINGULAR, (fl & 1) ? "Singular matrix" : "Singular matrix (reduced camera system)");
  }
  if (h->check_solve) {
    rc = check_solve_residual(h);
    if (rc) return rc;
  }
  h->have_trial = true;
  return MVBA_OK;
}

int mvba_commit(mvba_handle *h) {
  if (!h) return fail(MVBA_ERR_BADARG, "null handle");
  if (!h->have_trial) return fail(MVBA_ERR_STATE, "commit without a trial step");
  h->cur = 1 - h->cur;
  h->have_trial = false; h->linearized = false;
  h->stats.n_commit++;
  return MVBA_OK;
}

int mvba_set_parameter_map(mvba_handle *h, const int32_t *col, int32_t n_free) {
  if (!h) return fail(MVBA_ERR_BADARG, "null handle");
  MVBA_HIP(hipSetDevice(h->device));
  const int m = h->m, n9 = 9 * m;
  auto is_gauge = [&](int g) { return (g >= 3 && g <= 8) || g == 12 + h->gauge_axis; };
  if (!col) {
    h->mapped = false;
    h->have_trial = false;
    return MVBA_OK;
  }
  if (n_free < 0 || n_free > h->D)
    return fail(MVBA_ERR_BADARG, "mvba_set_parameter_map: n_free = " + std::to_string(n_free) + " must be in 0 .. 9 n_images - 7 = " + std::to_string(h->D));
  std::vector<int> cnt(n_free + 1, 0), first(n_free, -1);
  for (int g = 0; g < n9; ++g) {
    const int j = col[g];
    if (j < -1 || j >= n_free)
      return fail(MVBA_ERR_BADARG, "mvba_set_parameter_map: col[" + std::to_string(g) + "] = " + std::to_string(j) + " is neither -1 nor below n_free = " + std::to_string(n_free));
    if (j >= 0 && is_gauge(g))
      return fail(MVBA_ERR_BADARG, "mvba_set_parameter_map: col[" + std::to_string(g) + "] is a gauge slot and must be -1");
    if (j < 0) continue;
    if (first[j] < 0) first[j] = g;
    else if (g % 9 != first[j] % 9 || g % 9 > 2)
      return fail(MVBA_ERR_BADARG, "mvba_set_parameter_map: col[" + std::to_string(g) + "] ties slot " + std::to_string(g) + " to slot " + std::to_string(first[j]) +
                                       " (unknown " + std::to_string(j) + "): only the same intrinsic parameter (f, u or v) of different cameras can be tied");
    ++cnt[j];
  }
  for (int j = 0; j < n_free; ++j)
    if (!cnt[j]) return fail(MVBA_ERR_BADARG, "mvba_set_parameter_map: unknown " + std::to_string(j) + " has no parameter slot");
  bool is_default = n_free == h->D;
  for (int g = 0, j = 0; is_default && g < n9; ++g) is_default = col[g] == (is_gauge(g) ? -1 : j++);
  h->have_trial = false;
  if (is_default) {
    h->mapped = false;
    return MVBA_OK;
  }
  std::vector<int> ptr(n_free + 1, 0), mem;
  for (int j = 0; j < n_free; ++j) ptr[j + 1] = ptr[j] + cnt[j];
  mem.resize(std::max(ptr[n_free], 1));
  {
    std::vector<int> fill(ptr.begin(), ptr.end() - 1);
    for (int g = 0; g < n9; ++g)
      if (col[g] >= 0) mem[fill[col[g]]++] = g;
  }
  int U = 0;
  while (U < n_free && cnt[U] == 1) ++U;
  std::vector<int2> pairs;
  int max_cnt = 1;
  {
    std::vector<int> tied;
    for (int j = 0; j < n_free; ++j)
      if (cnt[j] > 1) { tied.push_back(j); max_cnt = std::max(max_cnt, cnt[j]); }
    for (size_t a = 0; a < tied.size(); ++a)
      for (size_t b = 0; b <= a; ++b) pairs.push_back(make_int2(tied[a], tied[b]));
  }
  const int nblk = std::min(64, (max_cnt + 7) / 8);
  int2 *d_pairs = nullptr;
  double *d_part = nullptr;
  if (!pairs.empty()) {
    int rc = h->mem.alloc(&d_pairs, pairs.size());
    if (!rc) rc = h->mem.alloc(&d_part, pairs.size() * (size_t)nblk);
    if (rc) {
      h->mem.release(d_pairs);
      return rc;
    }
  }
  if (!h->d_map_col) {
    int rc = h->mem.alloc(&h->d_map_col, (size_t)n9);
    if (!rc) rc = h->mem.alloc(&h->d_map_ptr, (size_t)h->D + 1);
    if (!rc) rc = h->mem.alloc(&h->d_map_mem, (size_t)n9);
    if (!rc) rc = h->mem.alloc(&h->d_map_x, (size_t)n9 + 16);
    if (rc) {
      h->mem.release(h->d_map_col); h->mem.release(h->d_map_ptr); h->mem.release(h->d_map_mem); h->mem.release(h->d_map_x);
      h->mem.release(d_pairs); h->mem.release(d_part);
      return rc;
    }
  }
  MVBA_HIP(hipStreamSynchronize(h->stream));
  h->mem.release(h->d_map_pairs);
  h->mem.release(h->d_map_part);
  h->d_map_pairs = d_pairs;
  h->d_map_part = d_part;
  h->n_map_pairs = (int)pairs.size();
  h->map_nblk = nblk;
  if (!pairs.empty()) MVBA_HIP(hipMemcpy(h->d_map_pairs, pairs.data(), sizeof(int2) * pairs.size(), hipMemcpyHostToDevice));
  MVBA_HIP(hipMemcpy(h->d_map_col, col, sizeof(int) * n9, hipMemcpyHostToDevice));
  MVBA_HIP(hipMemcpy(h->d_map_ptr, ptr.data(), sizeof(int) * (n_free + 1), hipMemcpyHostToDevice));
  MVBA_HIP(hipMemcpy(h->d_map_mem, mem.data(), sizeof(int) * mem.size(), hipMemcpyHostToDevice));
  h->map_col.assign(col, col + n9);
  h->map_ptr = ptr;
  h->map_mem = mem;
  h->n_free = n_free;
  h->map_ld = (n_free + 3) & ~3;
  h->map_U = U;
  h->mapped = true;
  return MVBA_OK;
}

int mvba_residuals(mvba_handle *h, double *e) {
  if (!h || !e) return fail(MVBA_ERR_BADARG, "null argument");
  if (!h->have_params) return fail(MVBA_ERR_STATE, "no parameters set");
  MVBA_HIP(hipSetDevice(h->device));
  if (!h->nobs) return MVBA_OK;
  if (!h->d_resid) {
    int rc = h->mem.alloc(&h->d_resid, h->nobs);
    if (rc) return rc;
  }
  const size_t lds = h->gcam ? 0 : (size_t)h->m * CAM_LDS * sizeof(double);
  cam_tables(h, h->d_cam15[h->cur], nullptr);
  const unsigned grid = (unsigned)std::min<long long>(4096, (h->nobs + 255) / 256);
  hipLaunchKernelGGL(h->gcam ? k_residuals<true> : k_residuals<false>, dim3(grid), dim3(256), lds, h->stream, h->nobs, h->m,
                     (const double *)h->d_cam15[h->cur], (const double *)h->d_X[h->cur], (const int *)h->d_obs_pt, (const int *)h->d_cam,
                     (const double2 *)h->d_xy, h->f0, h->d_resid, (const double *)h->d_cam18);
  MVBA_HIP(hipGetLastError());
  MVBA_HIP(hipMemcpyAsync(e, h->d_resid, sizeof(double2) * h->nobs, hipMemcpyDeviceToHost, h->stream));
  MVBA_HIP(hipStreamSynchronize(h->stream));
  return MVBA_OK;
}

int mvba_covariance(mvba_handle *h, double *point_cov, double *cam_cov, double *cam_cov_full, double *timings_ms) {
  if (!h) return fail(MVBA_ERR_BADARG, "null handle");
  if (h->loss != LOSS_SQUARED)
    return fail(MVBA_ERR_BADARG, "mvba_covariance: the covariance is defined for the squared loss only (this engine has a robust loss)");
  if (!h->have_params) return fail(MVBA_ERR_STATE, "no parameters set");
  MVBA_HIP(hipSetDevice(h->device));
  const int m = h->m, D = h->solve_D(), ld = h->solve_ld(), nt = (D + NB - 1) / NB;
  const size_t n_sig = sig_block(m, m, m);
  auto free_cov = [&]() {
    for (double **q : {&h->d_cov_sig, &h->d_cov_panel, &h->d_cov_pts, &h->d_cov_cam}) h->mem.release(*q);
  };
  int local_rc = MVBA_OK;
  if (!h->d_cov_sig || !h->d_cov_panel || !h->d_cov_pts || !h->d_cov_cam) {
    free_cov();
    local_rc = h->mem.alloc(&h->d_cov_sig, n_sig);
    if (!local_rc) local_rc = h->mem.alloc(&h->d_cov_panel, 2 * (size_t)h->D * NB);
    if (!local_rc) local_rc = h->mem.alloc(&h->d_cov_pts, 6 * (size_t)h->N);
    if (!local_rc) local_rc = h->mem.alloc(&h->d_cov_cam, 81 * (size_t)m);
    if (local_rc) free_cov();
  }
  hipEvent_t ev[5] = {};
  struct EvFree { hipEvent_t *e; ~EvFree() { for (int i = 0; i < 5; ++i) if (e[i]) hipEventDestroy(e[i]); } } ev_free{ev};
  for (auto &e : ev)
    if (!local_rc && hipEventCreate(&e) != hipSuccess) local_rc = fail(MVBA_ERR_HIP, "hipEventCreate failed");
  const int mv = (D + 6) / 9 + 1;
  if (!local_rc && h->mapped && D > 0 && !h->d_cov_sigv) local_rc = h->mem.alloc(&h->d_cov_sigv, n_sig);
  const bool sharded = h->comm || h->host_ar;
  if (local_rc && !sharded) return local_rc;
  const std::string local_err = local_rc ? g_err : std::string();
  double *d_b = h->d_Ab + strip_offset(m, m);
  if (!local_rc) {
    MVBA_HIP(hipEventRecord(ev[0], h->stream));
    if (h->nobs) launch_resid_jac(h);
    h->linearized = true; h->have_trial = false;
    launch_point_inv(h, 0.0);
    launch_schur(h, 0.0);
    MVBA_HIP(hipGetLastError());
  } else {
    MVBA_HIP(hipMemsetAsync(d_b + 3, 0xFF, sizeof(double), h->stream));
  }
  {
    int rc = allreduce_Ab(h, false);
    if (rc) return rc;
  }
  if (sharded) {
    double mark = 0.0;
    MVBA_HIP(hipMemcpyAsync(&mark, d_b + 3, sizeof(double), hipMemcpyDeviceToHost, h->stream));
    MVBA_HIP(hipStreamSynchronize(h->stream));
    if (local_rc) return fail(local_rc, local_err);
    if (std::isnan(mark))
      return fail(MVBA_ERR_HIP, "mvba_covariance: another rank could not allocate its covariance buffers (or the reduced system is not finite)");
  }
  MVBA_HIP(hipEventRecord(ev[1], h->stream));
  if (D > 0) launch_factor(h);
  MVBA_HIP(hipEventRecord(ev[2], h->stream));
  if (D > 0)
  hipLaunchKernelGGL(k_cov_assemble, dim3(nt), dim3(256), 0, h->stream, h->d_Ared, ld, D, (const double *)h->d_Ztiles,
                     (const double *)h->d_Lblk);
  double *panel[2] = {h->d_cov_panel, h->d_cov_panel + (size_t)D * NB};
  for (int J = nt - 1; J >= 0; --J) {
    const int grid = (nt - 1 - J) + (J >= 1 ? nt - J : 0);
    if (grid)
      hipLaunchKernelGGL(k_cov_trtri, dim3(grid), dim3(256), 0, h->stream, h->d_Ared, ld, D, nt, J, (const double *)panel[J & 1],
                         panel[(J + 1) & 1]);
  }
  MVBA_HIP(hipMemsetAsync(h->d_cov_sig, 0, sizeof(double) * n_sig, h->stream));
  if (h->mapped) {
    if (D > 0) {
      hipLaunchKernelGGL(k_cov_lauum, dim3(nt * (nt + 1) / 2), dim3(256), 0, h->stream, (const double *)h->d_Ared, ld, D, nt, mv,
                         h->gauge_axis, h->d_cov_sigv);
      hipLaunchKernelGGL(k_map_cov_expand, dim3((unsigned)((81 * m + 255) / 256), m), dim3(256), 0, h->stream, m, mv, h->gauge_axis,
                         (const int *)h->d_map_col, (const double *)h->d_cov_sigv, h->d_cov_sig);
    }
  } else
  hipLaunchKernelGGL(k_cov_lauum, dim3(nt * (nt + 1) / 2), dim3(256), 0, h->stream, (const double *)h->d_Ared, ld, D, nt, m,
                     h->gauge_axis, h->d_cov_sig);
  MVBA_HIP(hipEventRecord(ev[3], h->stream));
  if (h->N && point_cov) {
    const double pairs = h->N ? 0.5 * ((double)h->nobs / (double)h->N) * ((double)h->nobs / (double)h->N + 1.0) : 0.0;
    const int G = pairs > 48.0 ? 64 : (pairs > 24.0 ? 32 : (pairs > 12.0 ? 16 : 8));
    const unsigned grid = (unsigned)std::min<long long>(8192, (h->N * G + 255) / 256);
    auto kern = G == 64 ? k_point_cov<64> : (G == 32 ? k_point_cov<32> : (G == 16 ? k_point_cov<16> : k_point_cov<8>));
    hipLaunchKernelGGL(kern, dim3(grid), dim3(256), 0, h->stream, h->N, m, (const long long *)h->d_pt_ptr, (const int *)h->d_cam,
                       (const double2 *)h->d_rec, (const double *)h->d_PL, (const double *)h->d_cov_sig, 1.0 / h->f0, h->d_cov_pts,
                       h->d_flag);
  }
  if (cam_cov)
    hipLaunchKernelGGL(k_cov_cam_diag, dim3((unsigned)((81LL * m + 255) / 256)), dim3(256), 0, h->stream, m,
                       (const double *)h->d_cov_sig, h->d_cov_cam);
  MVBA_HIP(hipGetLastError());
  MVBA_HIP(hipEventRecord(ev[4], h->stream));
  int fl = 0;
  MVBA_HIP(hipMemcpyAsync(&fl, h->d_flag, sizeof(int), hipMemcpyDeviceToHost, h->stream));
  MVBA_HIP(hipStreamSynchronize(h->stream));
  if (fl) {
    MVBA_HIP(hipMemsetAsync(h->d_flag, 0, sizeof(int), h->stream));
    MVBA_HIP(hipStreamSynchronize(h->stream));
    if (fl & (1 | COV_FLAG_POINT)) return fail(MVBA_ERR_SINGULAR, "Singular matrix (a point block E_a is singular: a point seen once, or without parallax)");
    return fail(MVBA_ERR_SINGULAR, "Singular matrix (the undamped reduced camera system is not positive definite)");
  }
  if (timings_ms)
    for (int i = 0; i < 4; ++i) {
      float ms = 0.f;
      MVBA_HIP(hipEventElapsedTime(&ms, ev[i], ev[i + 1]));
      timings_ms[i] = ms;
    }
  if (point_cov && h->N) MVBA_HIP(hipMemcpy(point_cov, h->d_cov_pts, sizeof(double) * 6 * h->N, hipMemcpyDeviceToHost));
  if (cam_cov) MVBA_HIP(hipMemcpy(cam_cov, h->d_cov_cam, sizeof(double) * 81 * m, hipMemcpyDeviceToHost));
  if (cam_cov_full) {
    std::vector<double> strip((size_t)SIG_BS * m);
    const size_t n9 = 9 * (size_t)m;
    for (int k = 0; k < m; ++k) {
      MVBA_HIP(hipMemcpy(strip.data(), h->d_cov_sig + sig_block(k, k, m), sizeof(double) * SIG_BS * (m - k), hipMemcpyDeviceToHost));
      for (int l = k; l < m; ++l) {
        const double *b = strip.data() + (size_t)SIG_BS * (l - k);
        for (int i = 0; i < 9; ++i)
          for (int j = 0; j < 9; ++j) {
            const double v = 2.0 * b[9 * i + j];
            cam_cov_full[(9 * (size_t)k + i) * n9 + 9 * (size_t)l + j] = v;
            cam_cov_full[(9 * (size_t)l + j) * n9 + 9 * (size_t)k + i] = v;
          }
      }
    }
  }
  return MVBA_OK;
}

namespace {
constexpr int SNAP_SLAB = 8;
size_t snap_stride(const mvba_handle *h) { return (3 * (size_t)h->N + (size_t)CAM_IN * h->m + 1) & ~(size_t)1; }
}

int mvba_snapshot(mvba_handle *h) {
  if (!h) return fail(MVBA_ERR_BADARG, "null handle");
  if (!h->have_params) return fail(MVBA_ERR_STATE, "no parameters set");
  MVBA_HIP(hipSetDevice(h->device));
  const size_t stride = snap_stride(h);
  const size_t slab = (size_t)(h->n_snap / SNAP_SLAB);
  if (slab >= h->snap_slabs.size()) {
    double *p = nullptr;
    int rc = h->mem.alloc(&p, stride * SNAP_SLAB);
    if (rc) return rc;
    h->snap_slabs.push_back(p);
  }
  double *dst = h->snap_slabs[slab] + stride * (size_t)(h->n_snap % SNAP_SLAB);
  MVBA_HIP(hipMemcpyAsync(dst, h->d_X[h->cur], sizeof(double) * 3 * h->N, hipMemcpyDeviceToDevice, h->stream));
  MVBA_HIP(hipMemcpyAsync(dst + 3 * h->N, h->d_cam15[h->cur], sizeof(double) * CAM_IN * h->m, hipMemcpyDeviceToDevice, h->stream));
  h->n_snap++;
  return MVBA_OK;
}

int mvba_snapshot_count(mvba_handle *h, int64_t *n) {
  if (!h || !n) return fail(MVBA_ERR_BADARG, "null argument");
  *n = h->n_snap;
  return MVBA_OK;
}

int mvba_snapshot_read(mvba_handle *h, int64_t i, double *X, double *f, double *u, double *t, double *R) {
  if (!h || !X || !f || !u || !t || !R) return fail(MVBA_ERR_BADARG, "null argument");
  if (i < 0 || i >= h->n_snap) return fail(MVBA_ERR_BADARG, "no such log entry");
  MVBA_HIP(hipSetDevice(h->device));
  const double *src = h->snap_slabs[(size_t)(i / SNAP_SLAB)] + snap_stride(h) * (size_t)(i % SNAP_SLAB);
  std::vector<double> cam((size_t)h->m * CAM_IN);
  MVBA_HIP(hipMemcpyAsync(X, src, sizeof(double) * 3 * h->N, hipMemcpyDeviceToHost, h->stream));
  MVBA_HIP(hipMemcpyAsync(cam.data(), src + 3 * h->N, sizeof(double) * cam.size(), hipMemcpyDeviceToHost, h->stream));
  MVBA_HIP(hipStreamSynchronize(h->stream));
  for (int k = 0; k < h->m; ++k) {
    const double *c = cam.data() + (size_t)k * CAM_IN;
    f[k] = c[0]; u[2 * k] = c[1]; u[2 * k + 1] = c[2];
    for (int q = 0; q < 3; ++q) t[3 * k + q] = c[3 + q];
    for (int q = 0; q < 9; ++q) R[9 * k + q] = c[6 + q];
  }
  return MVBA_OK;
}

int mvba_snapshot_restore(mvba_handle *h, int64_t i) {
  if (!h) return fail(MVBA_ERR_BADARG, "null handle");
  if (i < 0 || i >= h->n_snap) return fail(MVBA_ERR_BADARG, "no such log entry");
  MVBA_HIP(hipSetDevice(h->device));
  const double *src = h->snap_slabs[(size_t)(i / SNAP_SLAB)] + snap_stride(h) * (size_t)(i % SNAP_SLAB);
  MVBA_HIP(hipMemcpyAsync(h->d_X[h->cur], src, sizeof(double) * 3 * h->N, hipMemcpyDeviceToDevice, h->stream));
  MVBA_HIP(hipMemcpyAsync(h->d_cam15[h->cur], src + 3 * h->N, sizeof(double) * CAM_IN * h->m, hipMemcpyDeviceToDevice, h->stream));
  h->have_params = true; h->linearized = false; h->have_trial = false;
  return MVBA_OK;
}

int mvba_snapshot_clear(mvba_handle *h) {
  if (!h) return fail(MVBA_ERR_BADARG, "null handle");
  h->n_snap = 0;
  return MVBA_OK;
}

int mvba_set_profiling(mvba_handle *h, int32_t enabled) {
  if (!h) return fail(MVBA_ERR_BADARG, "null handle");
  h->profiling = enabled == 2 ? 2 : (enabled != 0);
  return MVBA_OK;
}

int mvba_get_stats(mvba_handle *h, mvba_stats *out) {
  if (!h || !out) return fail(MVBA_ERR_BADARG, "null argument");
  MVBA_HIP(hipSetDevice(h->device));
  int rc = sync_and_drain(h);
  if (rc) return rc;
  *out = h->stats;
  return MVBA_OK;
}

int mvba_get_info(mvba_handle *h, int64_t *out8) {
  if (!h || !out8) return fail(MVBA_ERR_BADARG, "null argument");
  out8[0] = h->n_items;
  out8[1] = h->n_items_offdiag;
  out8[2] = h->n_units;
  out8[3] = h->schur_mode;
  out8[4] = h->rccl_version;
  out8[5] = NCCL_VERSION_CODE;
  out8[6] = h->nranks;
  out8[7] = h->schur_mode == SCHUR_SLOTS ? h->n_slot_items : 0;
  return MVBA_OK;
}

int mvba_reset_stats(mvba_handle *h) {
  if (!h) return fail(MVBA_ERR_BADARG, "null handle");
  MVBA_HIP(hipSetDevice(h->device));
  int rc = sync_and_drain(h);
  if (rc) return rc;
  h->stats = mvba_stats{};
  return MVBA_OK;
}

int mvba_comm_unique_id(void *id128) {
  if (!id128) return fail(MVBA_ERR_BADARG, "null argument");
  static_assert(sizeof(ncclUniqueId) == 128, "ncclUniqueId size");
  if (int rc = rccl_load()) return rc;
  ncclUniqueId id;
  ncclResult_t r = g_rccl.GetUniqueId(&id);
  if (r != ncclSuccess) return fail(MVBA_ERR_RCCL, std::string("ncclGetUniqueId: ") + g_rccl.GetErrorString(r));
  memcpy(id128, &id, 128);
  return MVBA_OK;
}

int mvba_comm_init(mvba_handle *h, const void *id128, int32_t rank, int32_t n_ranks) {
  if (!h || !id128 || n_ranks < 1 || rank < 0 || rank >= n_ranks) return fail(MVBA_ERR_BADARG, "bad comm arguments");
  MVBA_HIP(hipSetDevice(h->device));
  if (int rc = rccl_load()) return rc;
  ncclUniqueId id;
  memcpy(&id, id128, 128);
  ncclResult_t r = g_rccl.CommInitRank(&h->comm, n_ranks, id, rank);
  if (r != ncclSuccess) return fail(MVBA_ERR_RCCL, std::string("ncclCommInitRank: ") + g_rccl.GetErrorString(r));
  h->rank = rank; h->nranks = n_ranks;
  h->rccl_version = g_rccl.version;
  int rc = h->mem.alloc(&h->d_allcost, 2 * (size_t)n_ranks);
  if (rc) return rc;
  MVBA_HIP(hipHostMalloc((void **)&h->h_allcost, 2 * sizeof(double) * n_ranks));
  return MVBA_OK;
}

int mvba_comm_init_host(mvba_handle *h, int32_t rank, int32_t n_ranks, mvba_host_allreduce_fn fn, void *user) {
  if (!h || !fn || n_ranks < 1 || rank < 0 || rank >= n_ranks) return fail(MVBA_ERR_BADARG, "bad comm arguments");
  if (h->comm) return fail(MVBA_ERR_STATE, "handle already has an RCCL communicator");
  h->host_ar = fn; h->host_ar_user = user;
  h->rank = rank; h->nranks = n_ranks;
  return MVBA_OK;
}

int mvba_debug_read(mvba_handle *h, int32_t which, double *out, int64_t capacity, int64_t *n) {
  if (!h || !n) return fail(MVBA_ERR_BADARG, "null argument");
  MVBA_HIP(hipSetDevice(h->device));
  const size_t n9 = 9 * (size_t)h->m;
  long long cnt = 0;
  switch (which) {
    case MVBA_BUF_RESIDUAL: cnt = 2 * h->nobs; break;
    case MVBA_BUF_JX: cnt = 6 * h->nobs; break;
    case MVBA_BUF_JC: cnt = 18 * h->nobs; break;
    case MVBA_BUF_E: cnt = 6 * h->N; break;
    case MVBA_BUF_DP: cnt = 3 * h->N; break;
    case MVBA_BUF_A_FULL: cnt = n9 * n9; break;
    case MVBA_BUF_B_FULL: cnt = n9; break;
    case MVBA_BUF_DXI: cnt = n9; break;
    case MVBA_BUF_DX: case MVBA_BUF_TRIAL_X: cnt = 3 * h->N; break;
    case MVBA_BUF_TRIAL_CAM: cnt = (long long)CAM_IN * h->m; break;
    case MVBA_BUF_INDEX_K: case MVBA_BUF_INDEX_L: case MVBA_BUF_INDEX_A:
      cnt = h->schur_mode == SCHUR_SLOTS ? h->n_slot_items : (h->schur_mode == SCHUR_PAIRS ? h->n_items : 0);
      break;
    case MVBA_BUF_INDEX_SEG: cnt = h->schur_mode == SCHUR_SLOTS ? (long long)h->n_waves * h->slot_nseg : 0; break;
    case MVBA_BUF_WEIGHT: cnt = h->nobs; break;
    default: return fail(MVBA_ERR_BADARG, "unknown buffer id");
  }
  *n = cnt;
  if (!out) return MVBA_OK;
  if (capacity < cnt) return fail(MVBA_ERR_BADARG, "output buffer too small");
  MVBA_HIP(hipStreamSynchronize(h->stream));
  auto d2h = [&](const void *src, size_t bytes) { return hipMemcpy(out, src, bytes, hipMemcpyDeviceToHost); };
  if (which == MVBA_BUF_RESIDUAL || which == MVBA_BUF_JX || which == MVBA_BUF_JC) {
    std::vector<double> r((size_t)2 * REC * h->nobs);
    MVBA_HIP(hipMemcpy(r.data(), h->d_rec, sizeof(double) * r.size(), hipMemcpyDeviceToHost));
    std::vector<double> sw;
    if (h->loss != LOSS_SQUARED && which == MVBA_BUF_JC) {
      sw.resize(h->nobs);
      MVBA_HIP(hipMemcpy(sw.data(), h->d_sqw, sizeof(double) * sw.size(), hipMemcpyDeviceToHost));
    }
    for (long long o = 0; o < h->nobs; ++o) {
      const double cu = sw.empty() ? 1.0 / h->f0 : sw[o] / h->f0;
      const double *q = r.data() + (size_t)o * 2 * REC;
      if (which == MVBA_BUF_RESIDUAL) {
        out[2 * o] = q[14]; out[2 * o + 1] = q[15];
      } else if (which == MVBA_BUF_JX) {
        for (int rr = 0; rr < 2; ++rr) for (int i = 0; i < 3; ++i) out[6 * o + 3 * rr + i] = q[2 * i + rr];
      } else {
        double *jc = out + 18 * o;
        for (int rr = 0; rr < 2; ++rr) {
          jc[9 * rr + 0] = q[6 + rr];
          jc[9 * rr + 1] = rr == 0 ? cu : 0.0;
          jc[9 * rr + 2] = rr == 1 ? cu : 0.0;
          for (int i = 0; i < 3; ++i) jc[9 * rr + 3 + i] = -q[2 * i + rr];
          for (int i = 0; i < 3; ++i) jc[9 * rr + 6 + i] = q[8 + 2 * i + rr];
        }
      }
    }
  } else if (which == MVBA_BUF_WEIGHT) {
    if (h->loss != LOSS_SQUARED) MVBA_HIP(d2h(h->d_sqw, sizeof(double) * h->nobs));
    else for (long long o = 0; o < h->nobs; ++o) out[o] = 1.0;
  } else if (which == MVBA_BUF_E || which == MVBA_BUF_DP) {
    std::vector<double> pl(9 * (size_t)h->N);
    MVBA_HIP(hipMemcpy(pl.data(), h->d_PL, sizeof(double) * pl.size(), hipMemcpyDeviceToHost));
    for (long long a = 0; a < h->N; ++a) {
      if (which == MVBA_BUF_E) for (int i = 0; i < 6; ++i) out[6 * a + i] = pl[9 * a + i];
      else for (int i = 0; i < 3; ++i) out[3 * a + i] = pl[9 * a + 6 + i];
    }
  } else if (which == MVBA_BUF_A_FULL) {
    const int m = h->m;
    std::vector<double> pk(strip_offset(m, m));
    MVBA_HIP(hipMemcpy(pk.data(), h->d_Ab, sizeof(double) * pk.size(), hipMemcpyDeviceToHost));
    for (size_t r = 0; r < n9; ++r)
      for (size_t cc = 0; cc < n9; ++cc) {
        const size_t lo = std::min(r, cc), hi = std::max(r, cc);
        const int k = (int)(lo / 9), l = (int)(hi / 9);
        const size_t rr = (k == l) ? r : lo, c2 = (k == l) ? cc : hi;
        out[r * n9 + cc] = pk[strip_offset(k, m) + (rr - 9 * k) * (size_t)(9 * (m - k)) + (c2 - 9 * k)];
      }
  } else if (which == MVBA_BUF_B_FULL) {
    MVBA_HIP(d2h(h->d_Ab + strip_offset(h->m, h->m), sizeof(double) * cnt));
  } else if (which == MVBA_BUF_DXI) {
    MVBA_HIP(d2h(h->d_dxi, sizeof(double) * cnt));
  } else if (which == MVBA_BUF_DX) {
    MVBA_HIP(d2h(h->d_dX, sizeof(double) * cnt));
  } else if (which == MVBA_BUF_TRIAL_X) {
    MVBA_HIP(d2h(h->d_X[1 - h->cur], sizeof(double) * cnt));
  } else if (which == MVBA_BUF_TRIAL_CAM) {
    MVBA_HIP(d2h(h->d_cam15[1 - h->cur], sizeof(double) * cnt));
  } else if (which >= MVBA_BUF_INDEX_K && which <= MVBA_BUF_INDEX_SEG) {
    if (h->schur_mode == SCHUR_SLOTS && which != MVBA_BUF_INDEX_SEG) {
      const long long n_steps = cnt / PSTEP;
      std::vector<int> tmp((size_t)n_steps * SLOT_IDX);
      if (cnt) MVBA_HIP(hipMemcpy(tmp.data(), h->d_it_x, sizeof(int) * tmp.size(), hipMemcpyDeviceToHost));
      const int off = which == MVBA_BUF_INDEX_K ? 0 : (which == MVBA_BUF_INDEX_L ? PSTEP : 2 * PSTEP);
      for (long long st = 0; st < n_steps; ++st)
        for (int sl = 0; sl < PSTEP; ++sl) out[st * PSTEP + sl] = (double)tmp[(size_t)st * SLOT_IDX + off + sl];
      return MVBA_OK;
    }
    const int *src = which == MVBA_BUF_INDEX_K ? h->d_it_k : (which == MVBA_BUF_INDEX_L ? h->d_it_l : (which == MVBA_BUF_INDEX_A ? h->d_it_a : h->d_seg_end));
    std::vector<int> tmp((size_t)cnt);
    if (cnt) MVBA_HIP(hipMemcpy(tmp.data(), src, sizeof(int) * tmp.size(), hipMemcpyDeviceToHost));
    for (long long i = 0; i < cnt; ++i) out[i] = (double)tmp[i];
  }
  return MVBA_OK;
}

int mvba_project(const double *X, int64_t n_points, const double *K, const double *R, const double *t, int32_t n_images,
                 const int64_t *pt_ptr, const int32_t *cam_idx, int64_t n_obs, double *xy, int32_t device) {
  if (!X || !K || !R || !t || !xy) return fail(MVBA_ERR_BADARG, "null argument");
  if (n_points < 0 || n_images < 1 || n_obs < 0 || (pt_ptr && !cam_idx)) return fail(MVBA_ERR_BADARG, "bad sizes");
  if (!pt_ptr && n_obs != n_points * (int64_t)n_images) return fail(MVBA_ERR_BADARG, "dense grid needs n_obs = n_points * n_images");
  if (n_points >= (1LL << 31)) return fail(MVBA_ERR_BADARG, "n_points must be < 2^31");
  if ((size_t)n_images * 12 * sizeof(double) > 160 * 1024 - 256) return fail(MVBA_ERR_BADARG, "too many cameras for the LDS camera table (max 1704)");
  if (n_obs == 0) return MVBA_OK;
  if (device >= 0) MVBA_HIP(hipSetDevice(device));
  std::vector<int> obs_pt;
  if (pt_ptr) {
    if (pt_ptr[0] != 0 || pt_ptr[n_points] != n_obs) return fail(MVBA_ERR_BADARG, "pt_ptr does not span n_obs");
    obs_pt.resize(n_obs);
    for (int64_t a = 0; a < n_points; ++a)
      for (int64_t o = pt_ptr[a]; o < pt_ptr[a + 1]; ++o) {
        if (cam_idx[o] < 0 || cam_idx[o] >= n_images) return fail(MVBA_ERR_BADARG, "cam_idx out of range");
        obs_pt[o] = (int)a;
      }
  }
  double *dX = nullptr, *dK = nullptr, *dR = nullptr, *dt = nullptr;
  double2 *dxy = nullptr;
  int *dpt = nullptr, *dcam = nullptr;
  DevBufs tmp;
#define PRJ(x) do { hipError_t e_ = (x); if (e_ != hipSuccess) return fail(MVBA_ERR_HIP, std::string(#x) + ": " + hipGetErrorString(e_)); } while (0)
  PRJ(hipMalloc((void **)&dX, sizeof(double) * 3 * std::max<int64_t>(n_points, 1))); tmp.own(dX);
  PRJ(hipMalloc((void **)&dK, sizeof(double) * 9 * n_images)); tmp.own(dK);
  PRJ(hipMalloc((void **)&dR, sizeof(double) * 9 * n_images)); tmp.own(dR);
  PRJ(hipMalloc((void **)&dt, sizeof(double) * 3 * n_images)); tmp.own(dt);
  PRJ(hipMalloc((void **)&dxy, sizeof(double2) * n_obs)); tmp.own(dxy);
  PRJ(hipMemcpy(dX, X, sizeof(double) * 3 * n_points, hipMemcpyHostToDevice));
  PRJ(hipMemcpy(dK, K, sizeof(double) * 9 * n_images, hipMemcpyHostToDevice));
  PRJ(hipMemcpy(dR, R, sizeof(double) * 9 * n_images, hipMemcpyHostToDevice));
  PRJ(hipMemcpy(dt, t, sizeof(double) * 3 * n_images, hipMemcpyHostToDevice));
  if (pt_ptr) {
    PRJ(hipMalloc((void **)&dpt, sizeof(int) * n_obs)); tmp.own(dpt);
    PRJ(hipMalloc((void **)&dcam, sizeof(int) * n_obs)); tmp.own(dcam);
    PRJ(hipMemcpy(dpt, obs_pt.data(), sizeof(int) * n_obs, hipMemcpyHostToDevice));
    PRJ(hipMemcpy(dcam, cam_idx, sizeof(int) * n_obs, hipMemcpyHostToDevice));
  }
  const int lds = (int)(sizeof(double) * 12 * n_images);
  PRJ(hipFuncSetAttribute((const void *)k_project_obs, hipFuncAttributeMaxDynamicSharedMemorySize, lds));
  const int grid = (int)std::max<int64_t>(1, std::min<int64_t>(2048, (n_obs + 255) / 256));
  hipLaunchKernelGGL(k_project_obs, dim3(grid), dim3(256), lds, 0, (long long)n_obs, n_images, dX, dK, dR, dt, dpt, dcam, dxy);
  PRJ(hipGetLastError());
  PRJ(hipMemcpy(xy, dxy, sizeof(double2) * n_obs, hipMemcpyDeviceToHost));
#undef PRJ
  return MVBA_OK;
}

int mvba_host_obs_math(const double *X3, const double *cam15, const double *xy2, double f0, double *out26) {
  if (!X3 || !cam15 || !xy2 || !out26) return fail(MVBA_ERR_BADARG, "null argument");
  alignas(16) double c[CAM_LDS];
  expand_cam(cam15, f0, c);
  ObsJ J;
  obs_math(X3[0], X3[1], X3[2], c, xy2[0], xy2[1], f0, J);
  out26[0] = J.e0; out26[1] = J.e1;
  for (int r = 0; r < 2; ++r) for (int i = 0; i < 3; ++i) out26[2 + 3 * r + i] = J.jx[r][i];
  for (int r = 0; r < 2; ++r) for (int i = 0; i < 9; ++i) out26[8 + 9 * r + i] = J.jc[r][i];
  return MVBA_OK;
}

}

#include "mvba_init.h"
#include "mvba_twoview.h"
```

### 3d-reconstruction-from-multi-view-exp_amd/csrc/mvba_create.h

```cpp

__global__ __launch_bounds__(256) void k_xy_from_planes(const double2 *__restrict__ planes, long long N, int m, double2 *__restrict__ xy) {
  const long long a = (long long)blockIdx.x * 256 + threadIdx.x;
  const int k = blockIdx.y;
  if (a < N) xy[a * m + k] = planes[(long long)k * N + a];
}

#define CR(x) do { int rc_ = (x); if (rc_) return rc_; } while (0)
#define CRH(x) do { hipError_t e_ = (x); if (e_ != hipSuccess) return fail(MVBA_ERR_HIP, std::string(#x) + ": " + hipGetErrorString(e_)); } while (0)

struct CreateTimer {
  bool on;
  std::chrono::steady_clock::time_point t_last = std::chrono::steady_clock::now();
  void lap(const char *what) {
    if (!on) return;
    const auto now = std::chrono::steady_clock::now();
    fprintf(stderr, "mvba_create: %-28s %8.1f ms\n", what, std::chrono::duration<double, std::milli>(now - t_last).count());
    t_last = now;
  }
};

int validate_problem(const mvba_problem *p, std::vector<int> &obs_pt) {
  if (p->n_points < 0 || p->n_images < 2 || p->n_obs < 0 || !p->pt_ptr || (p->n_obs && (!p->cam_idx || !p->xy)))
    return fail(MVBA_ERR_BADARG, "bad problem sizes or null arrays (need n_images >= 2)");
  if (p->gauge_axis != 0 && p->gauge_axis != 1) return fail(MVBA_ERR_BADARG, "gauge_axis must be 0 or 1");
// ... 302 lines not shown
  }
  for (const std::vector<int> *src : {&diag_lists, &off_lists})
    for (size_t first = 0; first < src->size(); first += PSTEP) {
      for (int sl = 0; sl < PSTEP; ++sl) wl.push_back(first + sl < src->size() ? (*src)[first + sl] : -1);
      sw.w_isdiag.push_back(src == &diag_lists);
    }
  const long long n_waves = sw.n_waves = (long long)sw.w_isdiag.size() * nR;
  ix.wdesc.assign(n_waves, make_int4(0, 0, 0, 0));
  ix.wunits.assign((size_t)n_waves * PSTEP, -1);
  sw.w_steps.assign(n_waves, 0);
  sw.w_beg.assign(n_waves + 1, 0);
  sw.sl_beg.assign((size_t)n_waves * PSTEP, 0);
  sw.sl_len.assign((size_t)n_waves * PSTEP, 0);
  for (long long b = 0; b < n_waves; ++b) {
    const int *vs = wl.data() + (size_t)(b / nR) * PSTEP;
    const int r = (int)(b % nR);
    for (int sl = 0; sl < PSTEP; ++sl) {
      const int id = vs[sl] >= 0 ? uid[(size_t)vs[sl] * nR + r] : -1;
      ix.wunits[(size_t)b * PSTEP + sl] = id;
      if (id < 0) continue;
      sw.sl_beg[(size_t)b * PSTEP + sl] = ((long long)ix.units[id].y << 32) | (unsigned)ix.units[id].x;
      sw.sl_len[(size_t)b * PSTEP + sl] = ix.units[id].z;
    }
  }
  for (int r = 0; r < nR; ++r)
    sw.nSeg = std::max<long long>(sw.nSeg, (in.p->pt_ptr[plan.R.lo[r + 1]] - in.p->pt_ptr[plan.R.lo[r]] + SLOT_SEG - 1) / SLOT_SEG);
  ix.seg_end.assign((size_t)n_waves * sw.nSeg, 0);
  ix.slot_nseg = sw.nSeg;
  return sw;
}

int upload_range_o0(const IndexInput &in, const PointRanges &R, DevBufs &engine, SchurIndex &ix) {
  std::vector<long long> ro0(R.nR);
  for (int r = 0; r < R.nR; ++r) ro0[r] = in.p->pt_ptr[R.lo[r]];
  CR(engine.alloc(&ix.d_range_o0, (size_t)R.nR));
  CRH(hipMemcpy(ix.d_range_o0, ro0.data(), sizeof(long long) * R.nR, hipMemcpyHostToDevice));
  return MVBA_OK;
}

int place_slot_steps(const SchurPlan &plan, SlotWaves &sw, const SchurIndex &ix, long long &total_steps) {
  for (long long b = 0; b < sw.n_waves; ++b) sw.w_beg[b + 1] = sw.w_beg[b] + sw.w_steps[b];
  total_steps = sw.w_beg[sw.n_waves];
  if (total_steps * PSTEP >= (1LL << 40)) return fail(MVBA_ERR_BADARG, "too many (point, camera pair) items");
  const size_t need = (size_t)total_steps * PSTEP * 12 + (size_t)total_steps * SLOT_IDX * 4 + ix.seg_end.size() * 4;
  size_t fr = 0, tot = 0;
  if (hipMemGetInfo(&fr, &tot) == hipSuccess && need > fr)
    return fail(MVBA_ERR_BADARG, "the slot-form Schur index needs " + std::to_string(need >> 20) + " MiB (" + std::to_string(total_steps * PSTEP) + " step rows for " +
                                     std::to_string(plan.L.T) + " items: " + std::to_string(plan.R.nR) + " ranges, skew " + std::to_string(SLOT_SKEW) + "), " +
                                     std::to_string(fr >> 20) + " MiB of device memory are free: use MVBA_SCHUR=pairs");
  return MVBA_OK;
}

void finish_slot_waves(const PointRanges &R, const SlotWaves &sw, long long total_steps, SchurIndex &ix) {
  const int nR = R.nR;
  std::vector<int> live(nR, 0);
  for (long long b = 0; b < sw.n_waves; ++b) live[b % nR] += sw.w_steps[b] > 0;
  for (long long b = 0; b < sw.n_waves; ++b) {
    const long long beg = sw.w_beg[b];
    ix.wdesc[b] = make_int4((int)(beg & 0xffffffffLL), (int)(beg >> 32), (int)sw.w_steps[b],
                            (sw.w_isdiag[b / nR] ? 1 : 0) | (live[b % nR] << 8));
  }
  ix.n_waves = (int)sw.n_waves;
  ix.slot_nR = nR;
  ix.n_slot_items = total_steps * PSTEP;
}

int count_pairs_host(const IndexInput &in, std::vector<long long> &cnt) {
  const mvba_problem *p = in.p;
  const int m = in.m, n_thr = in.n_thr;
  on_threads(n_thr, [&](int tid) {
    for (long long a = 0; a < in.N; ++a) {
      const int *cb = p->cam_idx + p->pt_ptr[a];
      const int d = (int)(p->pt_ptr[a + 1] - p->pt_ptr[a]);
      for (int i = 0; i < d; ++i) {
        if (cb[i] % n_thr != tid) continue;
        long long *row = cnt.data() + pair_id(m, cb[i], cb[i]) - cb[i];
        for (int j = i; j < d; ++j) row[cb[j]]++;
      }
    }
  });
  return MVBA_OK;
}

int build_index_host(const IndexInput &in, const SchurPlan &plan, DevBufs &engine, SchurIndex &ix, CreateTimer &timer) {
  const mvba_problem *p = in.p;
  const PairLists &L = plan.L;
  const PointRanges &R = plan.R;
  const long long N = in.N, P = in.P;
  const int m = in.m, n_thr = in.n_thr, nR = R.nR;
  std::vector<int> &it_k = ix.it_k, &it_l = ix.it_l, &it_a = ix.it_a;
  it_k.resize(L.T); it_l.resize(L.T); it_a.resize(L.T);
  {
    std::vector<long long> run(P, 0);
    on_threads(n_thr, [&](int tid) {
      for (long long a = 0; a < N; ++a) {
        const long long o0 = p->pt_ptr[a];
        const int *cb = p->cam_idx + o0;
        const int d = (int)(p->pt_ptr[a + 1] - o0);
        for (int i = 0; i < d; ++i) {
          if (cb[i] % n_thr != tid) continue;
          const long long rowp = pair_id(m, cb[i], cb[i]) - cb[i];
          for (int j = i; j < d; ++j) {
            const long long q = rowp + cb[j], r = run[q]++;
            const int sI = (int)(r % L.S[q]);
            const long long pos = L.vp_off[L.vp_ptr[q] + sI] + r / L.S[q];
            it_k[pos] = (int)(o0 + i); it_l[pos] = (int)(o0 + j); it_a[pos] = (int)a;
          }
        }
      }
    });
  }
  timer.lap("items sorted by pair");
  std::vector<int> uid;
  number_units(in, plan, [&](int v, int r) {
    auto before = [](int a, long long key) { return (long long)a < key; };
    return (long long)(std::lower_bound(it_a.data() + L.vp_off[v], it_a.data() + L.vp_off[v + 1], R.lo[r], before) - it_a.data());
  }, ix, uid);
  timer.lap("units");
  if (plan.mode == SCHUR_SLOTS) {
    SlotWaves sw = make_slot_waves(in, plan, uid, ix);
    const int nSeg = sw.nSeg;
    std::vector<int> st_k, st_l, st_a;
    auto merge = [&](long long b, long long base, bool fill) {
      const int r = (int)(b % nR);
      long long cur[PSTEP], end[PSTEP];
      for (int sl = 0; sl < PSTEP; ++sl) {
        cur[sl] = sw.sl_beg[(size_t)b * PSTEP + sl];
        end[sl] = cur[sl] + sw.sl_len[(size_t)b * PSTEP + sl];
      }
      long long steps = 0;
      const long long o_lo = p->pt_ptr[R.lo[r]];
      int sg = 0;
      auto key_of = [&](int sl) { return p->pt_ptr[it_a[cur[sl]]]; };
      while (true) {
        long long lo = -1;
        for (int sl = 0; sl < PSTEP; ++sl)
          if (cur[sl] < end[sl] && (lo < 0 || key_of(sl) < lo)) lo = key_of(sl);
        if (fill && lo >= 0)
          while (sg < nSeg && lo >= o_lo + (sg + 1) * SLOT_SEG) ix.seg_end[(size_t)b * nSeg + sg++] = (int)steps;
        if (lo < 0) break;
        for (int sl = 0; sl < PSTEP; ++sl) {
          const bool take = cur[sl] < end[sl] && key_of(sl) <= lo + SLOT_SKEW;
          if (fill) {
            const long long o = (base + steps) * PSTEP + sl;
            if (take) { st_k[o] = (int)(it_k[cur[sl]] - o_lo); st_l[o] = (int)(it_l[cur[sl]] - o_lo); st_a[o] = it_a[cur[sl]]; }
            else { st_k[o] = st_l[o] = 0; st_a[o] = (int)N; }
          }
          if (take) ++cur[sl];
        }
        ++steps;
      }
      if (fill)
        while (sg < nSeg) ix.seg_end[(size_t)b * nSeg + sg++] = (int)steps;
      return steps;
    };
    CR(upload_range_o0(in, R, engine, ix));
    on_threads(n_thr, [&](int tid) {
      for (long long b = tid; b < sw.n_waves; b += n_thr) sw.w_steps[b] = merge(b, 0, false);
    });
    timer.lap("slot merge (count)");
    long long total_steps = 0;
    CR(place_slot_steps(plan, sw, ix, total_steps));
    st_k.resize(total_steps * PSTEP); st_l.resize(total_steps * PSTEP); st_a.resize(total_steps * PSTEP);
    on_threads(n_thr, [&](int tid) {
      for (long long b = tid; b < sw.n_waves; b += n_thr)
        if (sw.w_steps[b]) merge(b, sw.w_beg[b], true);
    });
    timer.lap("slot merge (fill)");
    finish_slot_waves(R, sw, total_steps, ix);
    it_k.swap(st_k); it_l.swap(st_l); it_a.swap(st_a);
  } else {
    build_work_queues(in, plan, uid, ix);
  }
  return MVBA_OK;
}

struct DeviceIndexBuild {
  DevBufs mem;
  bool hist_lds = true;
  int idx_chunk = 32;
  long long idx_waves = 0;
  size_t idx_lds = 0;
  int *d_hist = nullptr;
  long long *d_cnt = nullptr;
};

int count_pairs_device(const IndexInput &in, const CreateKnobs &knobs, DeviceIndexBuild &dv, std::vector<long long> &cnt) {
  const long long N = in.N, P = in.P;
  dv.hist_lds = (size_t)P * sizeof(int) * IDX_WAVES <= 150 * 1024 && !knobs.index_global;
  const long long max_idx_waves = dv.hist_lds ? 4096 : std::max<long long>(IDX_WAVES, std::min<long long>(4096, (2LL << 30) / (4 * P)));
  dv.idx_chunk = (int)std::max<long long>(32, (N + max_idx_waves - 1) / max_idx_waves);
  dv.idx_waves = ((N + dv.idx_chunk - 1) / dv.idx_chunk + IDX_WAVES - 1) / IDX_WAVES * IDX_WAVES;
  dv.idx_lds = dv.hist_lds ? P * sizeof(int) * IDX_WAVES : 0;
  CR(dv.mem.alloc(&dv.d_hist, (size_t)dv.idx_waves * P));
  CR(dv.mem.alloc(&dv.d_cnt, (size_t)P));
  if (dv.hist_lds) {
    CRH(hipFuncSetAttribute((const void *)k_idx_count<false>, hipFuncAttributeMaxDynamicSharedMemorySize, (int)dv.idx_lds));
    CRH(hipFuncSetAttribute((const void *)k_idx_fill<false>, hipFuncAttributeMaxDynamicSharedMemorySize, (int)dv.idx_lds));
  } else {
    CRH(hipMemsetAsync(dv.d_hist, 0, sizeof(int) * (size_t)dv.idx_waves * P, in.stream));
  }
  hipLaunchKernelGGL(dv.hist_lds ? k_idx_count<false> : k_idx_count<true>, dim3((unsigned)(dv.idx_waves / IDX_WAVES)), dim3(64 * IDX_WAVES), dv.idx_lds,
                     in.stream, N, in.m, (int)P, in.d_pt_ptr, in.d_cam, dv.idx_chunk, dv.d_hist, (const int *)nullptr);
  hipLaunchKernelGGL(k_idx_scan, dim3((unsigned)((P + 255) / 256)), dim3(256), 0, in.stream, (int)P, (int)dv.idx_waves, dv.d_hist, dv.d_cnt);
  CRH(hipMemcpyAsync(cnt.data(), dv.d_cnt, sizeof(long long) * P, hipMemcpyDeviceToHost, in.stream));
  CRH(hipStreamSynchronize(in.stream));
  return MVBA_OK;
}

int build_index_device(const IndexInput &in, const SchurPlan &plan, DeviceIndexBuild &dv, DevBufs &engine, SchurIndex &ix, CreateTimer &timer) {
  const PairLists &L = plan.L;
  const PointRanges &R = plan.R;
  const long long N = in.N, P = in.P;
  const int m = in.m, nR = R.nR, VP = L.VP;
  hipStream_t stream = in.stream;
  DevBufs &tmp = dv.mem;
  int *d_pk = nullptr, *d_pl = nullptr, *d_pa = nullptr, *d_S = nullptr, *d_vp_ptr = nullptr;
  long long *d_vp_off = nullptr;
  CR(tmp.alloc(&d_pk, (size_t)L.T)); CR(tmp.alloc(&d_pl, (size_t)L.T)); CR(tmp.alloc(&d_pa, (size_t)L.T));
  CR(tmp.alloc(&d_S, (size_t)P)); CR(tmp.alloc(&d_vp_ptr, (size_t)P + 1)); CR(tmp.alloc(&d_vp_off, (size_t)VP + 1));
  CRH(hipMemcpyAsync(d_S, L.S.data(), sizeof(int) * P, hipMemcpyHostToDevice, stream));
  CRH(hipMemcpyAsync(d_vp_ptr, L.vp_ptr.data(), sizeof(int) * (P + 1), hipMemcpyHostToDevice, stream));
  CRH(hipMemcpyAsync(d_vp_off, L.vp_off.data(), sizeof(long long) * (VP + 1), hipMemcpyHostToDevice, stream));
  hipLaunchKernelGGL(dv.hist_lds ? k_idx_fill<false> : k_idx_fill<true>, dim3((unsigned)(dv.idx_waves / IDX_WAVES)), dim3(64 * IDX_WAVES), dv.idx_lds,
                     stream, N, m, (int)P, in.d_pt_ptr, in.d_cam, dv.idx_chunk, dv.d_hist, d_S, d_vp_ptr, d_vp_off, d_pk, d_pl, d_pa,
                     (const int *)nullptr);
  CRH(hipGetLastError());
  timer.lap("items sorted by pair");
  std::vector<long long> lo_tab((size_t)VP * (nR + 1));
  {
    long long *d_rl = nullptr, *d_lo = nullptr;
    CR(tmp.alloc(&d_rl, (size_t)nR + 1)); CR(tmp.alloc(&d_lo, lo_tab.size()));
    CRH(hipMemcpyAsync(d_rl, R.lo.data(), sizeof(long long) * (nR + 1), hipMemcpyHostToDevice, stream));
    const long long nt = (long long)lo_tab.size();
    hipLaunchKernelGGL(k_idx_bounds, dim3((unsigned)((nt + 255) / 256)), dim3(256), 0, stream, VP, nR, d_vp_off, d_rl, d_pa, d_lo, (const int *)nullptr);
    CRH(hipMemcpyAsync(lo_tab.data(), d_lo, sizeof(long long) * nt, hipMemcpyDeviceToHost, stream));
    CRH(hipStreamSynchronize(stream));
    tmp.release(d_rl); tmp.release(d_lo);
  }
  std::vector<int> uid;
  number_units(in, plan, [&](int v, int r) { return lo_tab[(size_t)v * (nR + 1) + r]; }, ix, uid);
  timer.lap("units");
  if (plan.mode == SCHUR_SLOTS) {
    SlotWaves sw = make_slot_waves(in, plan, uid, ix);
    const long long n_waves = sw.n_waves;
    const int nSeg = sw.nSeg;
    CR(upload_range_o0(in, R, engine, ix));
    long long *d_slbeg = nullptr, *d_wbeg = nullptr;
    int *d_sllen = nullptr, *d_wsteps = nullptr;
    CR(tmp.alloc(&d_slbeg, sw.sl_beg.size())); CR(tmp.alloc(&d_sllen, sw.sl_len.size()));
    CR(tmp.alloc(&d_wsteps, (size_t)n_waves)); CR(tmp.alloc(&d_wbeg, (size_t)n_waves + 1));
    CRH(hipMemcpyAsync(d_slbeg, sw.sl_beg.data(), sizeof(long long) * sw.sl_beg.size(), hipMemcpyHostToDevice, stream));
    CRH(hipMemcpyAsync(d_sllen, sw.sl_len.data(), sizeof(int) * sw.sl_len.size(), hipMemcpyHostToDevice, stream));
    hipLaunchKernelGGL(k_idx_merge<false>, dim3((unsigned)n_waves), dim3(64), 0, stream, n_waves, nR, nSeg, SLOT_SKEW, SLOT_SEG, d_slbeg, d_sllen,
                       ix.d_range_o0, d_pk, d_pl, d_pa, d_wbeg, 0, (int)N, d_wsteps, (int *)nullptr, (int *)nullptr, (int *)nullptr,
                       (int *)nullptr, (const long long *)in.d_pt_ptr);
    std::vector<int> ws32(n_waves);
    CRH(hipMemcpyAsync(ws32.data(), d_wsteps, sizeof(int) * n_waves, hipMemcpyDeviceToHost, stream));
    CRH(hipStreamSynchronize(stream));
    for (long long b = 0; b < n_waves; ++b) sw.w_steps[b] = ws32[b];
    timer.lap("slot merge (count)");
    long long total_steps = 0;
    CR(place_slot_steps(plan, sw, ix, total_steps));
    const size_t rows = (size_t)total_steps * PSTEP;
    CR(engine.alloc(&ix.d_it_k, rows)); CR(engine.alloc(&ix.d_it_l, rows)); CR(engine.alloc(&ix.d_it_a, rows));
    CR(engine.alloc(&ix.d_seg_end, ix.seg_end.size()));
    CRH(hipMemcpyAsync(d_wbeg, sw.w_beg.data(), sizeof(long long) * (n_waves + 1), hipMemcpyHostToDevice, stream));
    hipLaunchKernelGGL(k_idx_merge<true>, dim3((unsigned)n_waves), dim3(64), 0, stream, n_waves, nR, nSeg, SLOT_SKEW, SLOT_SEG, d_slbeg, d_sllen,
                       ix.d_range_o0, d_pk, d_pl, d_pa, d_wbeg, 0, (int)N, d_wsteps, ix.d_it_k, ix.d_it_l, ix.d_it_a, ix.d_seg_end, (const long long *)in.d_pt_ptr);
    CRH(hipGetLastError());
    CRH(hipStreamSynchronize(stream));
    timer.lap("slot merge (fill)");
    finish_slot_waves(R, sw, total_steps, ix);
  } else {
    build_work_queues(in, plan, uid, ix);
    engine.adopt(tmp, d_pk); engine.adopt(tmp, d_pl); engine.adopt(tmp, d_pa);
    ix.d_it_k = d_pk; ix.d_it_l = d_pl; ix.d_it_a = d_pa;
  }
  tmp.release_all();
  ix.on_device = true;
  return MVBA_OK;
}

int alloc_engine_buffers(mvba_handle *h, K1Tiles &t) {
  const long long N = h->N, nobs = h->nobs;
  const int m = h->m;
  h->cost_grid = (int)std::max<long long>(1, std::min<long long>(2048, (nobs + 255) / 256));
  h->n_partials = std::max(h->cost_grid, 4096);
  CR(h->mem.alloc(&h->d_obs_pt, nobs));
  CR(h->mem.alloc(&h->d_xy, nobs));
  h->n_tiles = (int)t.tiles.size() - 1;
  h->any_split = t.any_split;
  if (t.any_split) {
    t.tile_slot.resize(t.tiles.size(), -1);
    h->n_splits = (int)t.splits.size();
    CR(h->mem.alloc(&h->d_tile_slot, t.tile_slot.size()));
    CR(h->mem.alloc(&h->d_splits, t.splits.size()));
    CR(h->mem.alloc(&h->d_PLsplit, 9 * (size_t)t.n_split_slots));
    CRH(hipMemcpy(h->d_tile_slot, t.tile_slot.data(), sizeof(int) * t.tile_slot.size(), hipMemcpyHostToDevice));
    CRH(hipMemcpy(h->d_splits, t.splits.data(), sizeof(int4) * t.splits.size(), hipMemcpyHostToDevice));
  }
  CR(h->mem.alloc(&h->d_tiles, t.tiles.size()));
  for (int i = 0; i < 2; ++i) { CR(h->mem.alloc(&h->d_X[i], 3 * N)); CR(h->mem.alloc(&h->d_cam15[i], (size_t)CAM_IN * m)); }
  CR(h->mem.alloc(&h->d_rec, (size_t)REC * (nobs + 1)));
  if (h->loss != LOSS_SQUARED) {
    CR(h->mem.alloc(&h->d_sqw, nobs + 1));
    CRH(hipMemset(h->d_sqw, 0, sizeof(double) * (nobs + 1)));
  }
  CR(h->mem.alloc(&h->d_PL, 9 * N));
  CR(h->mem.alloc(&h->d_PB, (size_t)PBS * (N + 1)));
  CRH(hipMemset(h->d_rec + (size_t)REC * nobs, 0, sizeof(double2) * REC));
  CRH(hipMemset(h->d_PB + (size_t)PBS * N, 0, sizeof(double) * PBS));
  const size_t n9 = 9 * (size_t)m;
  CR(h->mem.alloc(&h->d_Ab, strip_offset(m, m) + n9));
  CR(h->mem.alloc(&h->d_Ared, (size_t)(h->D + 1) * h->ld));
  CR(h->mem.alloc(&h->d_Lblk, (size_t)((h->D + SBW - 1) / SBW) * SBW * SBW));
  CR(h->mem.alloc(&h->d_Ztiles, (size_t)((h->D + NB - 1) / NB) * NB * NB));
  CR(h->mem.alloc(&h->d_dxi, n9));
  CR(h->mem.alloc(&h->d_dX, 3 * N));
  CR(h->mem.alloc(&h->d_partials, h->n_partials));
  CR(h->mem.alloc(&h->d_cost, 2));
  CR(h->mem.alloc(&h->d_flag, 1));
  CR(h->mem.alloc(&h->d_bar, 1 + 4 * (size_t)((9 * m + SBW - 1) / SBW)));
  CRH(hipHostMalloc((void **)&h->h_cost, 4 * sizeof(double), hipHostMallocMapped));
  memset(h->h_cost, 0, 4 * sizeof(double));
  if (hipHostGetDevicePointer((void **)&h->d_mail, h->h_cost, 0) != hipSuccess) h->d_mail = nullptr;
  h->h_flag = reinterpret_cast<int *>(h->h_cost + 1);
  return MVBA_OK;
}

int upload_schur_index(mvba_handle *h, const SchurPlan &plan, SchurIndex &ix) {
  const int m = h->m;
  h->n_items = plan.L.T;
  h->n_items_offdiag = plan.L.T - plan.L.Tdiag;
  h->n_units = (int)ix.units.size();
  h->n_waves = ix.n_waves; h->slot_nR = ix.slot_nR; h->slot_nseg = ix.slot_nseg; h->n_slot_items = ix.n_slot_items;
  h->index_on_device = ix.on_device;
  h->d_range_o0 = ix.d_range_o0;
  if (ix.on_device) { h->d_it_k = ix.d_it_k; h->d_it_l = ix.d_it_l; h->d_it_a = ix.d_it_a; h->d_seg_end = ix.d_seg_end; }
  const size_t P1 = (size_t)m * (m + 1) / 2 + 1;
  if (!ix.on_device) { CR(h->mem.alloc(&h->d_it_k, ix.it_k.size())); CR(h->mem.alloc(&h->d_it_l, ix.it_l.size())); CR(h->mem.alloc(&h->d_it_a, ix.it_a.size())); }
  CR(h->mem.alloc(&h->d_units, ix.units.size())); CR(h->mem.alloc(&h->d_unit_ptr, P1));
  CR(h->mem.alloc(&h->d_q_ptr, 9)); CR(h->mem.alloc(&h->d_q_units, ix.q_units.size()));
  CR(h->mem.alloc(&h->d_wdesc, ix.wdesc.size())); CR(h->mem.alloc(&h->d_wunits, ix.wunits.size()));
  if (!ix.on_device) CR(h->mem.alloc(&h->d_seg_end, ix.seg_end.size()));
  CR(h->mem.alloc(&h->d_prog, (size_t)h->slot_nR * std::max(1, h->slot_nseg) * PACE_STRIDE));
  if (!ix.seg_end.empty() && !ix.on_device) CRH(hipMemcpy(h->d_seg_end, ix.seg_end.data(), sizeof(int) * ix.seg_end.size(), hipMemcpyHostToDevice));
  if (!ix.wdesc.empty()) {
    CRH(hipMemcpy(h->d_wdesc, ix.wdesc.data(), sizeof(int4) * ix.wdesc.size(), hipMemcpyHostToDevice));
    CRH(hipMemcpy(h->d_wunits, ix.wunits.data(), sizeof(int) * ix.wunits.size(), hipMemcpyHostToDevice));
  }
  CR(h->mem.alloc(&h->d_partial, (size_t)UNIT_STRIDE * ix.units.size()));
  if (!ix.it_k.empty()) {
    CRH(hipMemcpy(h->d_it_k, ix.it_k.data(), sizeof(int) * ix.it_k.size(), hipMemcpyHostToDevice));
    CRH(hipMemcpy(h->d_it_l, ix.it_l.data(), sizeof(int) * ix.it_l.size(), hipMemcpyHostToDevice));
    CRH(hipMemcpy(h->d_it_a, ix.it_a.data(), sizeof(int) * ix.it_a.size(), hipMemcpyHostToDevice));
  }
  if (!ix.it_k.empty() || ix.on_device) {
    if (h->schur_mode == SCHUR_PAIRS) {
      std::vector<int4> qdesc(ix.units.size());
      for (size_t i = 0; i < ix.q_units.size(); ++i) qdesc[i] = ix.units[ix.q_units[i]];
      CRH(hipMemcpy(h->d_units, qdesc.data(), sizeof(int4) * qdesc.size(), hipMemcpyHostToDevice));
      int mx = 0;
      for (int x = 0; x < 8; ++x) mx = std::max(mx, ix.q_ptr[x + 1] - ix.q_ptr[x]);
      h->q_max = mx;
    }
    if (!ix.q_units.empty()) CRH(hipMemcpy(h->d_q_units, ix.q_units.data(), sizeof(int) * ix.q_units.size(), hipMemcpyHostToDevice));
  }
  if (h->schur_mode == SCHUR_SLOTS && h->n_slot_items) {
    const long long n_steps = h->n_slot_items / PSTEP;
    CR(h->mem.alloc(&h->d_it_x, (size_t)n_steps * SLOT_IDX));
    hipLaunchKernelGGL(k_idx_interleave, dim3((unsigned)((n_steps * SLOT_IDX + 255) / 256)), dim3(256), 0, h->stream, n_steps, h->d_it_k, h->d_it_l,
                       h->d_it_a, h->d_it_x);
    CRH(hipGetLastError());
    CRH(hipStreamSynchronize(h->stream));
    h->mem.release(h->d_it_k); h->mem.release(h->d_it_l); h->mem.release(h->d_it_a);
  }
  CRH(hipMemcpy(h->d_unit_ptr, ix.unit_ptr.data(), sizeof(int) * P1, hipMemcpyHostToDevice));
  CRH(hipMemcpy(h->d_q_ptr, ix.q_ptr.data(), sizeof(int) * 9, hipMemcpyHostToDevice));
  CRH(hipMemset(h->d_partial, 0, sizeof(double) * UNIT_STRIDE * std::max<size_t>(ix.units.size(), 1)));
  return MVBA_OK;
}

int upload_engine(mvba_handle *h, const mvba_problem *p, const std::vector<int> &obs_pt, const K1Tiles &t, const SchurPlan &plan, SchurIndex &ix) {
  const long long N = h->N, nobs = h->nobs;
  const int m = h->m;
  if (nobs) {
    CRH(hipMemcpy(h->d_obs_pt, obs_pt.data(), sizeof(int) * nobs, hipMemcpyHostToDevice));
    if (p->xy_layout == 1) {
      DevBufs tmp;
      double2 *planes = nullptr;
      CRH(hipMalloc((void **)&planes, sizeof(double2) * nobs));
      tmp.own(planes);
      hipError_t e = hipMemcpy(planes, p->xy, sizeof(double2) * nobs, hipMemcpyHostToDevice);
      if (e == hipSuccess) {
        hipLaunchKernelGGL(k_xy_from_planes, dim3((unsigned)((N + 255) / 256), m), dim3(256), 0, 0, planes, N, m, h->d_xy);
        e = hipGetLastError();
        if (e == hipSuccess) e = hipDeviceSynchronize();
      }
      CRH(e);
    } else {
      CRH(hipMemcpy(h->d_xy, p->xy, sizeof(double2) * nobs, hipMemcpyHostToDevice));
    }
  }
  CRH(hipMemcpy(h->d_tiles, t.tiles.data(), sizeof(int) * t.tiles.size(), hipMemcpyHostToDevice));
  CRH(hipMemset(h->d_PL, 0, sizeof(double) * 9 * std::max<long long>(N, 1)));
  CRH(hipMemset(h->d_flag, 0, sizeof(int)));
  if (h->schur_mode == SCHUR_DENSE) {
    const int T = (9 * m + 15) / 16;
    int n_cu_dense = 256;
    hipDeviceGetAttribute(&n_cu_dense, hipDeviceAttributeMultiprocessorCount, h->device);
    h->dense_tiles = T * (T + 1) / 2 + m;
    h->dense_blocks = (int)std::max<long long>(1, std::min<long long>((N + dense_ch(T) - 1) / dense_ch(T), (long long)n_cu_dense * dense_wgs(T)));
    CR(h->mem.alloc(&h->d_dense_part, (size_t)h->dense_blocks * h->dense_tiles * 256));
    if (!plan.dense_obs.empty()) {
      CR(h->mem.alloc(&h->d_dense_obs, plan.dense_obs.size()));
      CRH(hipMemcpy(h->d_dense_obs, plan.dense_obs.data(), sizeof(int) * plan.dense_obs.size(), hipMemcpyHostToDevice));
    }
  }
  if (h->use_pairs) CR(upload_schur_index(h, plan, ix));
  return MVBA_OK;
}

int set_kernel_attributes(mvba_handle *h, const CreateKnobs &knobs) {
  const int m = h->m;
  const bool robust = h->loss != LOSS_SQUARED;
  auto set_lds = [](const void *f, size_t bytes) { return hipFuncSetAttribute(f, hipFuncAttributeMaxDynamicSharedMemorySize, (int)bytes); };
  const size_t cam_lds = cam_lds_bytes(m, h->gcam, true);
  if (h->gcam) { CR(h->mem.alloc(&h->d_cam18, (size_t)m * CAM_LDS)); CR(h->mem.alloc(&h->d_dxi10, (size_t)m * DXI_LDS)); }
  for (int G : {2, 4, 8})
    for (int bt : {256, 512, 1024}) {
      CRH(set_lds(backsub_kernel(G, bt, false).fn(false), cam_lds));
      if (robust) CRH(set_lds(backsub_kernel(G, bt, false).fn(true), cam_lds));
    }
  CRH(set_lds((const void *)k_chol_super, SUPER_LDS));
  CRH(set_lds((const void *)k_chol_backsolve_all<true>, BACKSOLVE_LDS));
  {
    int per_cu = 0;
    CRH(hipDeviceGetAttribute(&h->n_cu, hipDeviceAttributeMultiprocessorCount, h->device));
    CRH(hipOccupancyMaxActiveBlocksPerMultiprocessor(&per_cu, (const void *)k_chol_backsolve_all<true>, SUPER_THREADS, BACKSOLVE_LDS));
    h->chol_onepass = per_cu >= 1 && !knobs.chol_launches;
    h->trail64_min = knobs.trail64_min;
    h->barrier_polls = knobs.barrier_polls;
  }
  const size_t k1_lds = k1_lds_bytes(m, h->gcam, h->k1_threads);
  CRH(set_lds(resid_jac_kernel(h->gcam, h->loss).fn(false), k1_lds));
  CRH(set_lds(cost_kernel(false, h->loss).fn(false), cam_lds));
  CRH(set_lds((const void *)k_residuals<false>, cam_lds));
  if (robust) {
    CRH(set_lds(resid_jac_kernel(h->gcam, h->loss).fn(true), k1_lds));
    CRH(set_lds(cost_kernel(false, h->loss).fn(true), cam_lds));
  }
  if (h->schur_mode == SCHUR_DENSE) {
    const int T = (9 * m + 15) / 16;
    CRH(set_lds(dense_kernel(T, h->d_dense_obs != nullptr).fn(robust), dense_lds_bytes(T, 16 * T / 9)));
  }
  return MVBA_OK;
}

int build_engine(mvba_handle *h, const mvba_problem *p, const CreateKnobs &knobs, const std::vector<int> &obs_pt, K1Tiles &tiles, CreateTimer &timer) {
  const long long N = h->N, nobs = h->nobs;
  const int m = h->m;
  if (p->device >= 0) CRH(hipSetDevice(p->device));
  CRH(hipGetDevice(&h->device));
  CRH(hipStreamCreateWithFlags(&h->stream, hipStreamNonBlocking));
  CR(h->mem.alloc(&h->d_pt_ptr, N + 1));
  CR(h->mem.alloc(&h->d_cam, nobs));
  CRH(hipMemcpy(h->d_pt_ptr, p->pt_ptr, sizeof(long long) * (N + 1), hipMemcpyHostToDevice));
  if (nobs) CRH(hipMemcpy(h->d_cam, p->cam_idx, sizeof(int) * nobs, hipMemcpyHostToDevice));
  timer.lap("device, topology upload");
  h->k1_threads = k1_block_threads(m, h->gcam);

  const bool dev_build = N > 0 && nobs > 0 && !knobs.index_host;
  const IndexInput in{p, N, nobs, (long long)m * (m + 1) / 2, m,
                      (int)std::max(1u, std::min({std::thread::hardware_concurrency(), 16u, (unsigned)m})), h->stream, h->d_pt_ptr, h->d_cam};
  DeviceIndexBuild dv;
  SchurPlan plan;
  SchurIndex ix;
  CR(decide_schur_form(in, knobs, h->loss, h->device, [&](std::vector<long long> &cnt) {
    return dev_build ? count_pairs_device(in, knobs, dv, cnt) : count_pairs_host(in, cnt);
  }, plan, timer));
  h->schur_mode = plan.mode;
  h->use_pairs = plan.mode != SCHUR_DENSE;
  if (h->use_pairs) CR(dev_build ? build_index_device(in, plan, dv, h->mem, ix, timer) : build_index_host(in, plan, h->mem, ix, timer));
  timer.lap("queues / wave descriptors");

  CR(alloc_engine_buffers(h, tiles));
  timer.lap("allocations");
  CR(upload_engine(h, p, obs_pt, tiles, plan, ix));
  timer.lap("uploads");
  CR(set_kernel_attributes(h, knobs));
  timer.lap("attributes");
  return MVBA_OK;
}

int create_engine(const mvba_problem *p, int loss, double loss_b, mvba_handle **out) {
  if (!p || !out) return fail(MVBA_ERR_BADARG, "null argument");
  const CreateKnobs knobs = read_create_knobs();
  CreateTimer timer{knobs.timing};
  std::vector<int> obs_pt;
  CR(validate_problem(p, obs_pt));
  timer.lap("validate, obs_pt");
  K1Tiles tiles = build_k1_tiles(p);
  timer.lap("K1 tiles");

  mvba_handle *h = new mvba_handle();
  const int m = p->n_images;
  h->N = p->n_points; h->nobs = p->n_obs; h->m = m; h->gauge_axis = p->gauge_axis; h->f0 = p->f0; h->D = 9 * m - 7; h->ld = (h->D + 3) & ~3;
  h->loss = loss; h->loss_b = loss_b;
  h->gcam = m > LDS_CAMERAS;
  h->force_big = knobs.force_big;
  h->check_solve = knobs.check_solve;
  h->check_solve_tol = knobs.check_solve_tol;
  if (int rc = build_engine(h, p, knobs, obs_pt, tiles, timer)) {
    const std::string err = g_err;
    mvba_destroy(h);
    g_err = err;
    return rc;
  }
  *out = h;
  return MVBA_OK;
}

#undef CR
#undef CRH
```

Before: 424.9.

## Speculatively linearize the trial state, fusing cost into residual-Jacobian kernel

After each trial step, the residual-Jacobian kernel now runs at the trial parameters in place of the separate cost kernel. It accumulates the robust cost per block into partials, so it produces the trial cost and a full linearization together. A second set of rec/PL/sqw buffers is double-buffered alongside the parameter sets, and a later commit adopts the trial linearization so linearize can skip its own resid_jac launch. This trades an extra large buffer set and a heavier trial evaluation for removing one full pass over observations per accepted iteration. Rejected steps pay more than the plain cost kernel would.

```diff
diff --git a/3d-reconstruction-from-multi-view-exp_amd/csrc/mvba.hip b/3d-reconstruction-from-multi-view-exp_amd/csrc/mvba.hip
--- a/3d-reconstruction-from-multi-view-exp_amd/csrc/mvba.hip
+++ b/3d-reconstruction-from-multi-view-exp_amd/csrc/mvba.hip
@@ -79,6 +79,10 @@
   return v;
 }
 
+__device__ __forceinline__ double wave_uniform(double v) {
+  return __hiloint2double(__builtin_amdgcn_readfirstlane(__double2hiint(v)), __builtin_amdgcn_readfirstlane(__double2loint(v)));
+}
+
 __device__ __forceinline__ double block_sum(double v, double *s_red ) {
   v = wave_sum(v);
   const int lane = threadIdx.x & 63, w = threadIdx.x >> 6;
@@ -122,7 +126,7 @@
   long long nobs, int m, const double *__restrict__ cam15, const double *__restrict__ X, const int *__restrict__ obs_pt,   \
       const int *__restrict__ cam_idx, const double2 *__restrict__ xy, double f0, const int *__restrict__ tile_start,     \
       int n_tiles, double2 *__restrict__ rec, double *__restrict__ PL, const int *__restrict__ tile_slot,                 \
-      double *__restrict__ PLsplit, const double *__restrict__ gcam
+      double *__restrict__ PLsplit, const double *__restrict__ gcam, double *__restrict__ cost_partials
 struct LossArgs {
   double b;
   double *sqw;
@@ -140,6 +144,7 @@
     load_cams_to_lds(cam15, m, f0, s_cam);
     __syncthreads();
   }
+  double cost = 0.0;
   for (int tile = blockIdx.x * nwave + wave; tile < n_tiles; tile += gridDim.x * nwave) {
     const int ts0 = tile_start[tile], ts1 = tile_start[tile + 1];
     const bool split = ts0 < 0;
@@ -150,6 +155,7 @@
     const bool live = lane < n;
     int a = -1;
     double c9[9] = {0, 0, 0, 0, 0, 0, 0, 0, 0};
+    double rho = 0.0;
     if (live) {
       a = obs_pt[o];
       const int k = cam_idx[o];
@@ -157,9 +163,11 @@
       const double *Xa = X + 3 * (size_t)a;
       ObsJ J;
       obs_math(Xa[0], Xa[1], Xa[2], GCAM ? gcam + (size_t)k * CAM_LDS : s_cam + k * CAM_LDS, z.x, z.y, f0, J);
+      const double so = J.e0 * J.e0 + J.e1 * J.e1;
       if constexpr (LOSS != LOSS_SQUARED) {
         const LossArgs la = (robust, ...);
-        const double sw = loss_sqrt_w<LOSS>(J.e0 * J.e0 + J.e1 * J.e1, la.b);
+        rho = loss_rho<LOSS>(so, la.b);
+        const double sw = loss_sqrt_w<LOSS>(so, la.b);
         J.e0 *= sw;
         J.e1 *= sw;
 #pragma unroll
@@ -171,6 +179,8 @@
           for (int i = 6; i < 9; ++i) J.jc[rr][i] *= sw;
         }
         la.sqw[o] = sw;
+      } else {
+        rho = so;
       }
       double2 *row = stage + lane * REC;
       const int sw = lane & 7;
@@ -192,6 +202,7 @@
       c9[7] = 2.0 * (J.jx[0][1] * J.e0 + J.jx[1][1] * J.e1);
       c9[8] = 2.0 * (J.jx[0][2] * J.e0 + J.jx[1][2] * J.e1);
     }
+    cost = wave_uniform(cost + wave_sum(rho));
     wave_sync();
 #pragma unroll
     for (int q = 0; q < REC; ++q) {
@@ -225,6 +236,14 @@
       }
     }
     wave_sync();
+  }
+  if (lane == 0) contrib[0] = cost;
+  __syncthreads();
+  if (threadIdx.x == 0) {
+    const double *w0 = reinterpret_cast<const double *>(stage);
+    double t = 0.0;
+    for (int w = 0; w < nwave; ++w) t += w0[(size_t)w * (64 * REC * 2)];
+    cost_partials[blockIdx.x] = t;
   }
 }
 
@@ -2452,8 +2471,12 @@
   double *d_X[2] = {nullptr, nullptr}, *d_cam15[2] = {nullptr, nullptr};
   int cur = 0;
   bool have_params = false, linearized = false, have_trial = false;
-  double2 *d_rec = nullptr;
-  double *d_PL = nullptr, *d_PB = nullptr;
+  double2 *d_rec[2] = {nullptr, nullptr};
+  double *d_PL[2] = {nullptr, nullptr}, *d_PB = nullptr;
+  bool two_lin = false, two_lin_failed = false;
+  bool spec_ok = true;
+  bool trial_linearized = false;
+  bool lin_adopted = false;
   double *d_Ab = nullptr, *d_Ared = nullptr, *d_Ztiles = nullptr, *d_Lblk = nullptr, *d_dxi = nullptr, *d_dX = nullptr, *d_lu = nullptr;
   int *d_ipiv = nullptr;
   double *d_partials = nullptr, *d_cost = nullptr, *h_cost = nullptr;
@@ -2483,7 +2506,7 @@
   double *d_cov_sig = nullptr, *d_cov_panel = nullptr, *d_cov_pts = nullptr, *d_cov_cam = nullptr;
   int loss = LOSS_SQUARED;
   double loss_b = 0.0;
-  double *d_sqw = nullptr;
+  double *d_sqw[2] = {nullptr, nullptr};
   double2 *d_resid = nullptr;
   double *d_init_cams = nullptr;
   bool mapped = false;
@@ -2627,10 +2650,16 @@
 template <typename... A>
 LossKernel<A...> loss_kernel(void (*squared)(A...), void (*robust)(A..., LossArgs)) { return {squared, robust}; }
 
+int lin_set(const mvba_handle *h) { return h->two_lin ? h->cur : 0; }
+
+template <typename... A, typename... Args>
+void launch_loss_set(mvba_handle *h, int set, LossKernel<A...> k, dim3 grid, dim3 block, size_t lds, Args... args) {
+  if (h->loss != LOSS_SQUARED) hipLaunchKernelGGL(k.robust, grid, block, lds, h->stream, args..., LossArgs{h->loss_b, h->d_sqw[set]});
+  else hipLaunchKernelGGL(k.squared, grid, block, lds, h->stream, args...);
+}
 template <typename... A, typename... Args>
 void launch_loss(mvba_handle *h, LossKernel<A...> k, dim3 grid, dim3 block, size_t lds, Args... args) {
-  if (h->loss != LOSS_SQUARED) hipLaunchKernelGGL(k.robust, grid, block, lds, h->stream, args..., LossArgs{h->loss_b, h->d_sqw});
-  else hipLaunchKernelGGL(k.squared, grid, block, lds, h->stream, args...);
+  launch_loss_set(h, lin_set(h), k, grid, block, lds, args...);
 }
 
 auto resid_jac_kernel(bool gcam, int loss) {
@@ -2688,16 +2717,19 @@
 void cam_tables(mvba_handle *h, const double *cam15, const double *dxi) {
   if (h->gcam) hipLaunchKernelGGL(k_cam_tables, dim3((h->m + 255) / 256), dim3(256), 0, h->stream, h->m, cam15, dxi, h->f0, h->d_cam18, h->d_dxi10);
 }
+int launch_sum_partials(mvba_handle *h, int n) {
+  double *mail = cost_mail(h);
+  const unsigned long long seq = h->cost_seq;
+  hipLaunchKernelGGL(k_sum_partials, dim3(1), dim3(1024), 0, h->stream, h->d_partials, n, h->d_cost, h->d_flag, mail, seq);
+  MVBA_HIP(hipGetLastError());
+  return MVBA_OK;
+}
 int launch_cost(mvba_handle *h, const double *cam15, const double *X) {
   const size_t lds = cam_lds_bytes(h->m, h->gcam, false);
   cam_tables(h, cam15, nullptr);
   launch_loss(h, cost_kernel(h->gcam, h->loss), dim3(h->cost_grid), dim3(lds > 40 * 1024 ? 512 : 256), lds, h->nobs, h->m, cam15, X,
               h->d_obs_pt, h->d_cam, h->d_xy, h->f0, h->d_partials, h->d_cam18);
-  double *mail = cost_mail(h);
-  const unsigned long long seq = h->cost_seq;
-  hipLaunchKernelGGL(k_sum_partials, dim3(1), dim3(1024), 0, h->stream, h->d_partials, h->cost_grid, h->d_cost, h->d_flag, mail, seq);
-  MVBA_HIP(hipGetLastError());
-  return MVBA_OK;
+  return launch_sum_partials(h, h->cost_grid);
 }
 
 struct CreateKnobs {
@@ -2800,6 +2832,7 @@
   MVBA_HIP(hipMemcpyAsync(h->d_cam15[h->cur], cam.data(), sizeof(double) * cam.size(), hipMemcpyHostToDevice, h->stream));
   MVBA_HIP(hipStreamSynchronize(h->stream));
   h->have_params = true; h->linearized = false; h->have_trial = false;
+  h->trial_linearized = false; h->spec_ok = true;
   return MVBA_OK;
 }
 
@@ -2838,7 +2871,7 @@
                      h->d_cam15[h->cur], h->d_sim);
   MVBA_HIP(hipGetLastError());
   MVBA_HIP(hipStreamSynchronize(h->stream));
-  h->linearized = false; h->have_trial = false;
+  h->linearized = false; h->have_trial = false; h->trial_linearized = false;
   return MVBA_OK;
 }
 
@@ -2855,17 +2888,18 @@
 }
 
 namespace {
-void launch_resid_jac(mvba_handle *h) {
+int launch_resid_jac(mvba_handle *h, int st, int set) {
   const int kt = h->k1_threads;
-  cam_tables(h, h->d_cam15[h->cur], nullptr);
+  cam_tables(h, h->d_cam15[st], nullptr);
   const int wpb = kt / 64;
-  const int grid = std::max(1, std::min(2048 * 256 / kt, (h->n_tiles + wpb - 1) / wpb));
-  launch_loss(h, resid_jac_kernel(h->gcam, h->loss), dim3(grid), dim3(kt), k1_lds_bytes(h->m, h->gcam, kt), h->nobs, h->m, h->d_cam15[h->cur],
-              h->d_X[h->cur], h->d_obs_pt, h->d_cam, h->d_xy, h->f0, h->d_tiles, h->n_tiles, h->d_rec, h->d_PL,
-              h->d_tile_slot, h->d_PLsplit, h->d_cam18);
+  const int grid = std::max(1, std::min({2048 * 256 / kt, (h->n_tiles + wpb - 1) / wpb, h->n_partials}));
+  launch_loss_set(h, set, resid_jac_kernel(h->gcam, h->loss), dim3(grid), dim3(kt), k1_lds_bytes(h->m, h->gcam, kt), h->nobs, h->m,
+                  h->d_cam15[st], h->d_X[st], h->d_obs_pt, h->d_cam, h->d_xy, h->f0, h->d_tiles, h->n_tiles, h->d_rec[set], h->d_PL[set],
+                  h->d_tile_slot, h->d_PLsplit, h->d_cam18, h->d_partials);
   if (h->n_splits)
     hipLaunchKernelGGL(k_sum_split, dim3((9 * h->n_splits + 255) / 256), dim3(256), 0, h->stream, h->n_splits, h->d_splits,
-                       h->d_PLsplit, h->d_PL);
+                       h->d_PLsplit, h->d_PL[set]);
+  return grid;
 }
 
 void launch_point_inv(mvba_handle *h, double c) {
@@ -2873,7 +2907,7 @@
   const size_t n9 = 9 * (size_t)m, nA = strip_offset(m, m);
   const long long nAb = (long long)(nA + n9);
   const unsigned grid = (unsigned)std::max<long long>((h->N + 255) / 256, std::min<long long>((nAb + 1023) / 1024, 4096));
-  hipLaunchKernelGGL(k_point_inv, dim3(std::max(grid, 1u)), dim3(256), 0, h->stream, h->N, c, h->d_PL, h->d_PB, h->d_flag,
+  hipLaunchKernelGGL(k_point_inv, dim3(std::max(grid, 1u)), dim3(256), 0, h->stream, h->N, c, h->d_PL[lin_set(h)], h->d_PB, h->d_flag,
                      h->d_Ab, nAb, h->d_prog, (long long)h->slot_nR * h->slot_nseg * PACE_STRIDE,
                      h->schur_mode == SCHUR_DENSE ? 1 : 0);
 }
@@ -2887,14 +2921,14 @@
     if (h->schur_mode == SCHUR_SLOTS) {
       if (h->n_waves)
         hipLaunchKernelGGL(k_schur_slots, dim3(h->n_waves), dim3(64), SLOT_LDS, h->stream, h->d_wdesc,
-                           h->d_wunits, h->d_it_x, (const int *)nullptr, (const int *)nullptr, h->d_rec, h->d_PB, c, h->f0, h->d_partial,
+                           h->d_wunits, h->d_it_x, (const int *)nullptr, (const int *)nullptr, h->d_rec[lin_set(h)], h->d_PB, c, h->f0, h->d_partial,
                            h->slot_nR, h->d_seg_end, h->d_prog, h->slot_nseg, SLOT_LAG, h->d_range_o0);
     } else if (h->n_units) {
       auto launch = [&](auto kern, auto... robust) {
         hipLaunchKernelGGL(kern, dim3(8 * h->q_max), dim3(64), PAIRS_LDS, h->stream, h->d_units, h->d_q_ptr, h->d_q_units, h->d_it_k, h->d_it_l,
-                           h->d_it_a, h->d_rec, h->d_PB, c, h->f0, h->d_partial, robust...);
+                           h->d_it_a, h->d_rec[lin_set(h)], h->d_PB, c, h->f0, h->d_partial, robust...);
       };
-      if (h->loss != LOSS_SQUARED) launch(big ? k_schur_pairs_big_robust : k_schur_pairs_robust, (const double *)h->d_sqw);
+      if (h->loss != LOSS_SQUARED) launch(big ? k_schur_pairs_big_robust : k_schur_pairs_robust, (const double *)h->d_sqw[lin_set(h)]);
       else launch(big ? k_schur_pairs_big : k_schur_pairs);
     }
     hipLaunchKernelGGL(k_schur_reduce, dim3((unsigned)((long long)m * (m + 1) / 2)), dim3(128), 0, h->stream, m, h->d_unit_ptr,
@@ -2902,7 +2936,7 @@
   } else if (h->schur_mode == SCHUR_DENSE) {
     const int T = (9 * m + 15) / 16;
     launch_loss(h, dense_kernel(T, h->d_dense_obs != nullptr), dim3(h->dense_blocks), dim3(64 * (dense_consumers(T) + dense_ch(T))), dense_lds_bytes(T, m),
-                (const double2 *)h->d_rec, (const double *)h->d_PB, (const int *)h->d_dense_obs, (long long)h->N, m, 1.0 / h->f0, h->d_dense_part);
+                (const double2 *)h->d_rec[lin_set(h)], (const double *)h->d_PB, (const int *)h->d_dense_obs, (long long)h->N, m, 1.0 / h->f0, h->d_dense_part);
     const long long n_el = (long long)nA + 9 * m;
     hipLaunchKernelGGL(k_schur_dense_finish, dim3((unsigned)((n_el + 3) / 4)), dim3(256), 0, h->stream, m, T, h->dense_blocks,
                        (const double *)h->d_dense_part, c, d_A, d_b);
@@ -2974,12 +3008,12 @@
   if (!h) return fail(MVBA_ERR_BADARG, "null handle");
   if (!h->have_params) return fail(MVBA_ERR_STATE, "no parameters set");
   MVBA_HIP(hipSetDevice(h->device));
-  if (h->nobs) {
+  if (h->nobs && !(h->linearized && h->lin_adopted)) {
     Timed t(h, MVBA_K_RESID_JAC);
-    launch_resid_jac(h);
+    launch_resid_jac(h, h->cur, lin_set(h));
   }
   MVBA_HIP(hipGetLastError());
-  h->linearized = true; h->have_trial = false;
+  h->linearized = true; h->have_trial = false; h->trial_linearized = false; h->lin_adopted = false;
   h->stats.n_linearize++;
   return MVBA_OK;
 }
@@ -3049,7 +3083,32 @@
   return MVBA_OK;
 }
 
-int launch_tail_and_cost(mvba_handle *h, double *E_trial) {
+bool alloc_second_linearisation(mvba_handle *h) {
+  if (h->two_lin) return true;
+  if (h->two_lin_failed) return false;
+  double2 *rec = nullptr;
+  double *PL = nullptr, *sqw = nullptr;
+  const std::string err = g_err;
+  bool ok = h->mem.alloc(&rec, (size_t)REC * (h->nobs + 1)) == MVBA_OK && h->mem.alloc(&PL, 9 * (size_t)h->N) == MVBA_OK &&
+            (h->loss == LOSS_SQUARED || h->mem.alloc(&sqw, (size_t)h->nobs + 1) == MVBA_OK);
+  ok = ok && hipMemsetAsync(rec + (size_t)REC * h->nobs, 0, sizeof(double2) * REC, h->stream) == hipSuccess &&
+       hipMemsetAsync(PL, 0, sizeof(double) * 9 * std::max<long long>(h->N, 1), h->stream) == hipSuccess &&
+       (!sqw || hipMemsetAsync(sqw, 0, sizeof(double) * (h->nobs + 1), h->stream) == hipSuccess);
+  if (!ok) {
+    (void)hipGetLastError();
+    h->mem.release(rec); h->mem.release(PL); h->mem.release(sqw);
+    g_err = err;
+    h->two_lin_failed = true;
+    return false;
+  }
+  const int other = 1 - h->cur;
+  if (h->cur == 1) { h->d_rec[1] = h->d_rec[0]; h->d_PL[1] = h->d_PL[0]; h->d_sqw[1] = h->d_sqw[0]; }
+  h->d_rec[other] = rec; h->d_PL[other] = PL; h->d_sqw[other] = sqw;
+  h->two_lin = true;
+  return true;
+}
+
+int launch_tail_and_cost(mvba_handle *h, double *E_trial, bool spec) {
   const int m = h->m, trial = 1 - h->cur;
   {
     Timed t(h, MVBA_K_BACKSUB_COST);
@@ -3065,7 +3124,18 @@
       launch_loss(h, backsub_kernel(G, bt, h->gcam), dim3(nblk), dim3(bt), lds, h->N, m, h->d_pt_ptr, h->d_cam, h->d_PB, h->d_dxi,
                   h->d_X[h->cur], h->d_cam15[h->cur], h->f0, h->d_X[trial], h->d_dX, h->d_cam18, h->d_dxi10);
     }
-    int rc = launch_cost(h, h->d_cam15[trial], h->d_X[trial]);
+    if (!spec) {
+      int rc = launch_cost(h, h->d_cam15[trial], h->d_X[trial]);
+      if (rc) return rc;
+    }
+  }
+  if (spec) {
+    int n_part;
+    {
+      Timed t(h, MVBA_K_RESID_JAC);
+      n_part = launch_resid_jac(h, trial, 1 - lin_set(h));
+    }
+    int rc = launch_sum_partials(h, n_part);
     if (rc) return rc;
   }
   return global_cost(h, E_trial);
@@ -3119,6 +3189,9 @@
   if (!h || !E_trial) return fail(MVBA_ERR_BADARG, "null argument");
   if (!h->linearized) return fail(MVBA_ERR_STATE, "try_step before linearize");
   MVBA_HIP(hipSetDevice(h->device));
+  const bool spec = h->spec_ok && h->nobs > 0 && alloc_second_linearisation(h);
+  h->spec_ok = false;
+  h->trial_linearized = false;
   {
     Timed t(h, MVBA_K_POINT_INV);
     launch_point_inv(h, c);
@@ -3133,21 +3206,21 @@
   launch_solve(h, h->chol_onepass);
   MVBA_HIP(hipGetLastError());
   h->stats.n_try_step++;
-  rc = launch_tail_and_cost(h, E_trial);
+  rc = launch_tail_and_cost(h, E_trial, spec);
   if (rc) return rc;
   if ((*h->h_flag & 8) && !(*h->h_flag & 1)) {
     MVBA_HIP(hipMemsetAsync(h->d_flag, 0, sizeof(int), h->stream));
     h->chol_onepass = false;
     h->stats.n_barrier_fallback++;
     launch_solve(h, false);
-    rc = launch_tail_and_cost(h, E_trial);
+    rc = launch_tail_and_cost(h, E_trial, spec);
     if (rc) return rc;
   }
   if ((*h->h_flag & 2) && !(*h->h_flag & (1 | 8))) {
     rc = launch_lu_solve(h);
     if (rc) return rc;
     h->stats.n_lu_fallback++;
-    rc = launch_tail_and_cost(h, E_trial);
+    rc = launch_tail_and_cost(h, E_trial, spec);
     if (rc) return rc;
   }
   if (*h->h_flag) {
@@ -3161,6 +3234,7 @@
     if (rc) return rc;
   }
   h->have_trial = true;
+  h->trial_linearized = spec;
   return MVBA_OK;
 }
 
@@ -3168,7 +3242,8 @@
   if (!h) return fail(MVBA_ERR_BADARG, "null handle");
   if (!h->have_trial) return fail(MVBA_ERR_STATE, "commit without a trial step");
   h->cur = 1 - h->cur;
-  h->have_trial = false; h->linearized = false;
+  h->have_trial = false; h->linearized = h->trial_linearized; h->lin_adopted = h->trial_linearized;
+  h->trial_linearized = false; h->spec_ok = true;
   h->stats.n_commit++;
   return MVBA_OK;
 }
@@ -3323,8 +3398,8 @@
   double *d_b = h->d_Ab + strip_offset(m, m);
   if (!local_rc) {
     MVBA_HIP(hipEventRecord(ev[0], h->stream));
-    if (h->nobs) launch_resid_jac(h);
-    h->linearized = true; h->have_trial = false;
+    if (h->nobs) launch_resid_jac(h, h->cur, lin_set(h));
+    h->linearized = true; h->have_trial = false; h->trial_linearized = false; h->lin_adopted = false;
     launch_point_inv(h, 0.0);
     launch_schur(h, 0.0);
     MVBA_HIP(hipGetLastError());
@@ -3374,7 +3449,7 @@
     const unsigned grid = (unsigned)std::min<long long>(8192, (h->N * G + 255) / 256);
     auto kern = G == 64 ? k_point_cov<64> : (G == 32 ? k_point_cov<32> : (G == 16 ? k_point_cov<16> : k_point_cov<8>));
     hipLaunchKernelGGL(kern, dim3(grid), dim3(256), 0, h->stream, h->N, m, (const long long *)h->d_pt_ptr, (const int *)h->d_cam,
-                       (const double2 *)h->d_rec, (const double *)h->d_PL, (const double *)h->d_cov_sig, 1.0 / h->f0, h->d_cov_pts,
+                       (const double2 *)h->d_rec[lin_set(h)], (const double *)h->d_PL[lin_set(h)], (const double *)h->d_cov_sig, 1.0 / h->f0, h->d_cov_pts,
                        h->d_flag);
   }
   if (cam_cov)
@@ -3474,6 +3549,7 @@
   MVBA_HIP(hipMemcpyAsync(h->d_X[h->cur], src, sizeof(double) * 3 * h->N, hipMemcpyDeviceToDevice, h->stream));
   MVBA_HIP(hipMemcpyAsync(h->d_cam15[h->cur], src + 3 * h->N, sizeof(double) * CAM_IN * h->m, hipMemcpyDeviceToDevice, h->stream));
   h->have_params = true; h->linearized = false; h->have_trial = false;
+  h->trial_linearized = false; h->spec_ok = true;
   return MVBA_OK;
 }
 
@@ -3585,11 +3661,11 @@
   auto d2h = [&](const void *src, size_t bytes) { return hipMemcpy(out, src, bytes, hipMemcpyDeviceToHost); };
   if (which == MVBA_BUF_RESIDUAL || which == MVBA_BUF_JX || which == MVBA_BUF_JC) {
     std::vector<double> r((size_t)2 * REC * h->nobs);
-    MVBA_HIP(hipMemcpy(r.data(), h->d_rec, sizeof(double) * r.size(), hipMemcpyDeviceToHost));
+    MVBA_HIP(hipMemcpy(r.data(), h->d_rec[lin_set(h)], sizeof(double) * r.size(), hipMemcpyDeviceToHost));
     std::vector<double> sw;
     if (h->loss != LOSS_SQUARED && which == MVBA_BUF_JC) {
       sw.resize(h->nobs);
-      MVBA_HIP(hipMemcpy(sw.data(), h->d_sqw, sizeof(double) * sw.size(), hipMemcpyDeviceToHost));
+      MVBA_HIP(hipMemcpy(sw.data(), h->d_sqw[lin_set(h)], sizeof(double) * sw.size(), hipMemcpyDeviceToHost));
     }
     for (long long o = 0; o < h->nobs; ++o) {
       const double cu = sw.empty() ? 1.0 / h->f0 : sw[o] / h->f0;
@@ -3610,11 +3686,11 @@
       }
     }
   } else if (which == MVBA_BUF_WEIGHT) {
-    if (h->loss != LOSS_SQUARED) MVBA_HIP(d2h(h->d_sqw, sizeof(double) * h->nobs));
+    if (h->loss != LOSS_SQUARED) MVBA_HIP(d2h(h->d_sqw[lin_set(h)], sizeof(double) * h->nobs));
     else for (long long o = 0; o < h->nobs; ++o) out[o] = 1.0;
   } else if (which == MVBA_BUF_E || which == MVBA_BUF_DP) {
     std::vector<double> pl(9 * (size_t)h->N);
-    MVBA_HIP(hipMemcpy(pl.data(), h->d_PL, sizeof(double) * pl.size(), hipMemcpyDeviceToHost));
+    MVBA_HIP(hipMemcpy(pl.data(), h->d_PL[lin_set(h)], sizeof(double) * pl.size(), hipMemcpyDeviceToHost));
     for (long long a = 0; a < h->N; ++a) {
       if (which == MVBA_BUF_E) for (int i = 0; i < 6; ++i) out[6 * a + i] = pl[9 * a + i];
       else for (int i = 0; i < 3; ++i) out[3 * a + i] = pl[9 * a + 6 + i];
diff --git a/3d-reconstruction-from-multi-view-exp_amd/csrc/mvba_create.h b/3d-reconstruction-from-multi-view-exp_amd/csrc/mvba_create.h
--- a/3d-reconstruction-from-multi-view-exp_amd/csrc/mvba_create.h
+++ b/3d-reconstruction-from-multi-view-exp_amd/csrc/mvba_create.h
@@ -628,14 +628,14 @@
   }
   CR(h->mem.alloc(&h->d_tiles, t.tiles.size()));
   for (int i = 0; i < 2; ++i) { CR(h->mem.alloc(&h->d_X[i], 3 * N)); CR(h->mem.alloc(&h->d_cam15[i], (size_t)CAM_IN * m)); }
-  CR(h->mem.alloc(&h->d_rec, (size_t)REC * (nobs + 1)));
+  CR(h->mem.alloc(&h->d_rec[0], (size_t)REC * (nobs + 1)));
   if (h->loss != LOSS_SQUARED) {
-    CR(h->mem.alloc(&h->d_sqw, nobs + 1));
-    CRH(hipMemset(h->d_sqw, 0, sizeof(double) * (nobs + 1)));
-  }
-  CR(h->mem.alloc(&h->d_PL, 9 * N));
+    CR(h->mem.alloc(&h->d_sqw[0], nobs + 1));
+    CRH(hipMemset(h->d_sqw[0], 0, sizeof(double) * (nobs + 1)));
+  }
+  CR(h->mem.alloc(&h->d_PL[0], 9 * N));
   CR(h->mem.alloc(&h->d_PB, (size_t)PBS * (N + 1)));
-  CRH(hipMemset(h->d_rec + (size_t)REC * nobs, 0, sizeof(double2) * REC));
+  CRH(hipMemset(h->d_rec[0] + (size_t)REC * nobs, 0, sizeof(double2) * REC));
   CRH(hipMemset(h->d_PB + (size_t)PBS * N, 0, sizeof(double) * PBS));
   const size_t n9 = 9 * (size_t)m;
   CR(h->mem.alloc(&h->d_Ab, strip_offset(m, m) + n9));
@@ -730,7 +730,7 @@
     }
   }
   CRH(hipMemcpy(h->d_tiles, t.tiles.data(), sizeof(int) * t.tiles.size(), hipMemcpyHostToDevice));
-  CRH(hipMemset(h->d_PL, 0, sizeof(double) * 9 * std::max<long long>(N, 1)));
+  CRH(hipMemset(h->d_PL[0], 0, sizeof(double) * 9 * std::max<long long>(N, 1)));
   CRH(hipMemset(h->d_flag, 0, sizeof(int)));
   if (h->schur_mode == SCHUR_DENSE) {
     const int T = (9 * m + 15) / 16;
```

Result: no change. 426.4, median of 6 (+0.4%).
